# abdenlab/giql

Hardware: AMD Instinct MI355X
Metric: overlap-pairs/sec, 10Mx100M INTERSECTS inner join (higher is better)
Workload: dtype int32

## Files before the change

### giql_amd/csrc/giql_hip.hip

```cpp
#include <hip/hip_runtime.h>
#include <chrono>
#include <atomic>
#include <sys/mman.h>
#include <utility>
#if defined(__SSE2__)
#include <emmintrin.h>
#endif
#include <mutex>
#include <thread>
#include <stdarg.h>
#include <stdio.h>
#include <stdlib.h>
#include <string.h>

#include <vector>

#include "../../include/giql_hip.h"
#include "aux_kernels.hip.h"
#include "take_kernels.hip.h"
#include "select_kernels.hip.h"
#include "cluster_kernels.hip.h"
#include "disjoin_kernels.hip.h"
#include "contain_kernels.hip.h"
#include "dev_common.hip.h"
#include "join_kernels.hip.h"
#include "onesweep.hip.h"
#include "bucket_sort.hip.h"
#include "radix_sort.hip.h"
#include "scan.hip.h"
#include "probe_kernels.hip.h"

using namespace giql;

static thread_local char g_err[512] = "";

static int set_err(int code, const char* fmt, ...) {
  va_list ap;
  va_start(ap, fmt);
  vsnprintf(g_err, sizeof(g_err), fmt, ap);
  va_end(ap);
  return code;
}

#define HIP_TRY(expr)                                                                     \
  do {                                                                                    \
    hipError_t _e = (expr);                                                               \
    if (_e != hipSuccess)                                                                 \
      return set_err(GIQL_ERR_HIP, "%s failed: %s (%s:%d)", #expr, hipGetErrorString(_e), \
                     __FILE__, __LINE__);                                                 \
  } while (0)

#define GIQL_TRY(expr)      \
  do {                      \
    int _rc = (expr);       \
    if (_rc != GIQL_OK) return _rc; \
  } while (0)

#ifndef GIQL_RC_ITEMS
#define GIQL_RC_ITEMS 1
#endif
constexpr int RC_ITEMS_C2 = GIQL_RC_ITEMS;
#ifndef GIQL_FILL_ITEMS
#define GIQL_FILL_ITEMS 16
#endif
constexpr int FILL_ITEMS_C2 = GIQL_FILL_ITEMS;

#ifndef GIQL_STREAM_GRID
#define GIQL_STREAM_GRID 16384u
#endif

static inline size_t align_up(size_t x, size_t a) { return (x + a - 1) / a * a; }
static inline u32 cdiv(u64 a, u64 b) { return (u32)((a + b - 1) / b); }

struct SortBufs {
  u32* key[2];
  u32* end[2];
  u32* rid[2];
};

struct InnerState {
  SortBufs sa, sb;
  u32 nt1 = 0, nt2 = 0;
  int c1_items = C1_ITEMS_MAX;
  u32* wlo1 = nullptr;
  u64* c1_base = nullptr;
  bool c1_fill = false;
  u32 *lo1 = nullptr, *cnt1 = nullptr;
  u64* off1 = nullptr;
  u32* wlo2 = nullptr;
  u32* lo2 = nullptr;
  u32* cnt2 = nullptr;
  u64* off2 = nullptr;
  int uniform = 0;
};

constexpr size_t C1_SMALL_ROWS = (size_t)4 << 20;
constexpr u64 OVERLAP_MAX_ROWS = (u64)4 << 20;

struct Switches {
  bool classic_sort = false;
  int os_variant = 0;
  int os_order = 2;
  u32 os_help_after = OS_HELP_AFTER;
  int inject_timeout = 0;
  bool no_uniform = false;
  bool no_span_hist = false;
  bool no_coarse_b = false;
  double coarse_max_group_rows = 8.0;
  bool no_fuse_count = false;
  bool no_local_sort = false;
  u64 local_min_rows = 1u << 21;
  double local_min_bucket_rows = 300.0;
  double local_max_bucket_rows = 2800.0;
  bool no_narrow = false;
  int force_bits = 0;
};

struct Guesses {
  bool local_sort = true;
  int os_order = 2;
  int inject_timeout = 0;
  u64 last_span = 0;
  bool last_no_irr = false;
  bool nearest_two_sorts = false;
  int nearest_aligned = -1;
  bool spec_valid = false;
  int spec_form = 0;
  i64 spec_len = 0;
  bool spec_aligned = false;
  bool spec_fuse_len_ok = false;
  bool spec_sorted[2] = {false, false};
  bool row_spec_valid = false;
  i64 row_spec_len = 0;
  int spec_misses = 0;
  int local_resorts = 0;
  int order_fallbacks = 0;
};

struct CallState {
  bool prezeroed = false;
  bool first_unstable = false;
  u32* span_hist_dirty[2] = {nullptr, nullptr};
  int force_local = 0;
  int index_bits = 16;
  bool used_sorted[2] = {false, false};
  bool last_sort_local = false;
  int last_local_bits = 16;
  bool count_fused = false;
  bool bucket_join = false;
};

struct InnerPlan {
  bool planned = false;
  bool plan_is_join = false;
  bool swapped = false;
  int32_t* fuse_a = nullptr;
  int32_t* fuse_b = nullptr;
  u64 fuse_cap = 0;
  bool fuse_done = false;
  giql_side side_a, side_b;
  u32 n_a = 0, n_b = 0;
  int n_chrom = 0;
  u64 n_reg = 0, n_irr = 0, n_c1 = 0;
  InnerState inner;
  u32* irr_a_list = nullptr;
  u32* irr_b_list = nullptr;
  u64* irr_off = nullptr;
};

struct DisjoinPlan {
  bool planned = false;
  giql_side target;
  u64 total = 0;
  i64* chrom_base = nullptr;
  u64* off = nullptr;
  u32* lo_first = nullptr;
  u32* bp = nullptr;
  u64* n_bp = nullptr;
  u32* ncov = nullptr;
  u32* cbp = nullptr;
};

struct ContainPlan {
  bool planned = false;
  giql_side outer, inner;
  u32 n_o = 0, n_i = 0;
  int form = 0;
  u64 n_cand = 0;
  u64 n_reg = 0, n_irr = 0;
  u32 n_tiles = 0;
  SortBufs so, si;
  u32* lo = nullptr;
  u64* coff = nullptr;
  u32* ct_part = nullptr;
  u64* tile_off = nullptr;
  u32* irr_o_list = nullptr;
  u32* irr_i_list = nullptr;
  u64* irr_off = nullptr;
};

struct giql_hip_ctx {
  explicit giql_hip_ctx(const Switches& s) : sw(s) {
    guess.local_sort = !s.no_local_sort;
    guess.os_order = s.os_order;
    guess.inject_timeout = s.inject_timeout;
  }
  const Switches sw;
  Guesses guess;
  CallState call;
  InnerPlan plan;
  DisjoinPlan dj;
  ContainPlan ct;

  int device = 0;
  int n_cu = 256;
  char* arena = nullptr;
  size_t arena_cap = 0;
  DevMeta* d_meta = nullptr;
  DevMeta* h_meta = nullptr;
  u32* part = nullptr;
  size_t part_cap = 0;
  void* stage_out = nullptr;
  size_t stage_out_cap = 0;
  char* xplan = nullptr;
  size_t xplan_cap = 0;
  char* ct_buf = nullptr;
  size_t ct_buf_cap = 0;
  u64* d_scratch64 = nullptr;
  hipStream_t side_stream = nullptr;
  hipEvent_t ev_fork = nullptr, ev_join = nullptr;
  u32* bucket_qwin = nullptr;
  u32* bucket_bnd = nullptr;
  u32* bucket_big = nullptr;

  int profiling = 0;
  int profile_phase = GIQL_PH_SORT_SCATTER;
  std::vector<hipEvent_t> ev_pool;
  struct Span {
    int phase;
    hipEvent_t a, b;
  };
  std::vector<Span> spans;
  size_t ev_used = 0;
  giql_hip_stats stats;
};

struct Carver {
  char* base;
  size_t off = 0;
  template <typename T>
  T* take(size_t n) {
    off = align_up(off, 256);
    T* p = base ? reinterpret_cast<T*>(base + off) : nullptr;
    off += n * sizeof(T);
    return p;
  }
};

static int grow_buffer(void** buf, size_t* cap, size_t need, size_t want, hipStream_t stream, const char* what) {
  if (need <= *cap) return GIQL_OK;
  HIP_TRY(hipStreamSynchronize(stream));
  if (*buf) HIP_TRY(hipFree(*buf));
  *buf = nullptr;
  *cap = 0;
  const hipError_t e = hipMalloc(buf, want);
  if (e != hipSuccess)
    return set_err(GIQL_ERR_NOMEM, "hipMalloc(%zu bytes) for %s failed: %s", want, what, hipGetErrorString(e));
  *cap = want;
  return GIQL_OK;
}

static int ensure_arena(giql_hip_ctx* ctx, size_t bytes, hipStream_t stream) {
  if (bytes <= ctx->arena_cap) return GIQL_OK;
  ctx->plan.planned = false;
  ctx->dj.planned = false;
  ctx->ct.planned = false;
  const size_t want = align_up(bytes + bytes / 8, (size_t)1 << 20);
  GIQL_TRY(grow_buffer((void**)&ctx->arena, &ctx->arena_cap, bytes, want, stream, "the workspace"));
  if (getenv("GIQL_HIP_DEBUG_ADDR")) fprintf(stderr, "[giql_hip] arena %p + %zu bytes\n", (void*)ctx->arena, want);
  return GIQL_OK;
}

static int grow_part(giql_hip_ctx* ctx, size_t words, hipStream_t stream) {
  return grow_buffer((void**)&ctx->part, &ctx->part_cap, words * sizeof(u32), (words + words / 4) * sizeof(u32), stream,
                     "the fill partition");
}

template <typename Carve>
static int claim_arena(giql_hip_ctx* ctx, hipStream_t stream, Carve&& carve) {
  ctx->plan.planned = false;
  ctx->dj.planned = false;
  ctx->ct.planned = false;
  GIQL_TRY(ensure_arena(ctx, carve(nullptr), stream));
  carve(ctx->arena);
  return GIQL_OK;
}

struct Phase {
  giql_hip_ctx* ctx;
  hipStream_t stream;
  int phase;
  hipEvent_t a = nullptr, b = nullptr;
  Phase(giql_hip_ctx* c, hipStream_t s, int ph, int launches = 1) : ctx(c), stream(s), phase(ph) {
    ctx->stats.phase_launches[ph] += launches;
    if (!ctx->profiling || (ctx->profiling == 2 && ph != ctx->profile_phase)) return;
    while (ctx->ev_used + 2 > ctx->ev_pool.size()) {
      hipEvent_t e;
      if (hipEventCreate(&e) != hipSuccess) return;
      ctx->ev_pool.push_back(e);
    }
    a = ctx->ev_pool[ctx->ev_used++];
    b = ctx->ev_pool[ctx->ev_used++];
    (void)hipEventRecord(a, stream);
  }
  ~Phase() {
    if (!a) return;
    (void)hipEventRecord(b, stream);
    ctx->spans.push_back({phase, a, b});
  }
};

static void reset_stats(giql_hip_ctx* ctx) {
  memset(&ctx->stats, 0, sizeof(ctx->stats));
  ctx->call = CallState{};
  ctx->spans.clear();
  ctx->ev_used = 0;
}

static int begin_call(giql_hip_ctx* ctx) {
  HIP_TRY(hipSetDevice(ctx->device));
  ctx->ct.planned = false;
  reset_stats(ctx);
  return GIQL_OK;
}

static int check_side(const giql_side* s, const char* name);
static int begin_pair_call(giql_hip_ctx* ctx, const giql_side* a, const giql_side* b, int32_t n_chrom) {
  GIQL_TRY(check_side(a, "a"));
  GIQL_TRY(check_side(b, "b"));
  if (n_chrom < 0) return set_err(GIQL_ERR_INVALID, "n_chrom < 0");
  GIQL_TRY(begin_call(ctx));
  ctx->stats.n_a = a->n;
  ctx->stats.n_b = b->n;
  return GIQL_OK;
}

struct PrezeroGuard {
  giql_hip_ctx* c;
  ~PrezeroGuard() {
    c->call.prezeroed = false;
    c->call.first_unstable = false;
  }
};

struct ForceLocal {
  giql_hip_ctx* c;
  ForceLocal(giql_hip_ctx* ctx, int v) : c(ctx) { c->call.force_local = v; }
  ~ForceLocal() {
    c->call.force_local = 0;
    c->call.index_bits = 16;
  }
};

static void collect_spans(giql_hip_ctx* ctx) {
  if (!ctx->profiling) return;
  for (auto& s : ctx->spans) {
    float ms = 0.f;
    if (hipEventElapsedTime(&ms, s.a, s.b) == hipSuccess) ctx->stats.phase_ms[s.phase] += ms;
  }
  ctx->spans.clear();
  ctx->ev_used = 0;
  float t = 0.f;
  for (int i = 0; i < GIQL_PH_N; i++) t += ctx->stats.phase_ms[i];
  ctx->stats.total_ms = t;
  ctx->stats.profiled = 1;
}

static int check_side(const giql_side* s, const char* name) {
  if (!s) return set_err(GIQL_ERR_INVALID, "side %s is NULL", name);
  if (s->n < 0 || s->n > 0x7FFFFFF0ll)
    return set_err(GIQL_ERR_INVALID, "side %s: n=%lld outside [0, 2^31-16]", name, (long long)s->n);
  if (s->n > 0 && (!s->chrom || !s->start || !s->end))
    return set_err(GIQL_ERR_INVALID, "side %s: NULL column buffer", name);
  if (s->start_off < -1 || s->start_off > 0 || s->end_off < -1 || s->end_off > 1)
    return set_err(GIQL_ERR_INVALID, "side %s: canonical offsets (%d,%d) outside {0,-1}x{+1,0,-1}",
                   name, s->start_off, s->end_off);
  return GIQL_OK;
}

static SideView view_of(const giql_side& s) {
  SideView v;
  v.chrom = s.chrom;
  v.start = s.start;
  v.end = s.end;
  v.n = (u32)s.n;
  v.start_off = s.start_off;
  v.end_off = s.end_off;
  return v;
}

static int post_launch(const char* what) {
  hipError_t e = hipGetLastError();
  if (e != hipSuccess)
    return set_err(GIQL_ERR_HIP, "kernel launch failed in %s: %s", what, hipGetErrorString(e));
  return GIQL_OK;
}

template <typename TOut>
static int run_scan(giql_hip_ctx* ctx, hipStream_t st, int phase, const u32* in, u64 n, TOut* out,
                    u64* bsums, u64* total_out, u64* total_out2 = nullptr) {
  if (n == 0) {
    if (total_out) HIP_TRY(hipMemsetAsync(total_out, 0, sizeof(u64), st));
    if (total_out2) HIP_TRY(hipMemsetAsync(total_out2, 0, sizeof(u64), st));
    return GIQL_OK;
  }
  const u32 nb = cdiv(n, SCAN_TILE);
  Phase ph(ctx, st, phase, 3);
  hipLaunchKernelGGL(k_scan_reduce, dim3(nb), dim3(SCAN_NT), 0, st, in, n, bsums);
  hipLaunchKernelGGL(k_scan_spine, dim3(1), dim3(1024), 0, st, bsums, nb, total_out, total_out2);
  hipLaunchKernelGGL((k_scan_down<TOut>), dim3(nb), dim3(SCAN_NT), 0, st, in, n, bsums, out);
  return post_launch("scan");
}

static int run_scan_diff(giql_hip_ctx* ctx, hipStream_t st, int phase, u32* hi, u32* lo, u64 n, const u32* n_irr,
                         u64* out, u64* bsums, u64* total_out, u64* total_out2) {
  const u32 nb = cdiv(n, SCAN_TILE);
  Phase ph(ctx, st, phase, 3);
  hipLaunchKernelGGL(k_scan_reduce_diff, dim3(nb), dim3(SCAN_NT), 0, st, hi, lo, n, n_irr, bsums);
  hipLaunchKernelGGL(k_scan_spine, dim3(1), dim3(1024), 0, st, bsums, nb, total_out, total_out2);
  hipLaunchKernelGGL(k_scan_down_diff, dim3(nb), dim3(SCAN_NT), 0, st, hi, lo, n, n_irr, bsums, out);
  return post_launch("scan (bounds)");
}

static int run_scan_chain(giql_hip_ctx* ctx, hipStream_t st, int phase, const u32* hi, const u32* lo, u64 n,
                          const u32* n_irr, u64* out, u64* chain_status, u64* total_out2, u32* part, u32 tile_log2,
                          u32 part_cap) {
  const u32 nb = cdiv(n, SC_TILE);
  Phase ph(ctx, st, phase, 1);
  hipLaunchKernelGGL(k_scan_chain_diff, dim3(nb), dim3(SC_NT), 0, st, hi, lo, (u32)n, n_irr, chain_status,
                     reinterpret_cast<u32*>(chain_status + nb + 1), out, total_out2, part, tile_log2, part_cap);
  return post_launch("scan (chained)");
}

struct LinBufs {
  int* gmin;
  int* gmax;
  i64* chrom_base;
  u32* chrom_first;
  int* len_part;
  u32* abase = nullptr;
  u32* top_partial = nullptr;
  u32* top_partial2 = nullptr;
  u32* hist_partial2 = nullptr;
};

static inline int sort_local_bits(const giql_hip_ctx* ctx, size_t n);
static inline bool sort_is_local(const giql_hip_ctx* ctx, size_t n) { return sort_local_bits(ctx, n) != 0; }

static int run_spans(giql_hip_ctx* ctx, hipStream_t st, const giql_side& a, const giql_side& b,
                     int n_chrom, const LinBufs& lb, int hist_side = -1, u32* hist_partial = nullptr) {
  const bool hist = hist_side >= 0 && hist_partial && lb.abase && lb.top_partial &&
                    n_chrom <= MM_HIST_CHROMS && (hist_side ? b.n : a.n) > 0;
  const bool hist2 = hist && lb.hist_partial2 && lb.top_partial2 && ctx->call.prezeroed && (hist_side ? a.n : b.n) > 0;
  if (hist && !ctx->call.prezeroed) {
    HIP_TRY(hipMemsetAsync(hist_partial, 0, (size_t)LIN_HIST_REPLICAS * 1024 * sizeof(u32), st));
    HIP_TRY(hipMemsetAsync(lb.top_partial, 0, (size_t)LIN_HIST_REPLICAS * MM_TOP_WORDS * sizeof(u32), st));
  }
  Phase ph(ctx, st, GIQL_PH_SPAN, 4);
  hipLaunchKernelGGL(k_init_minmax, dim3(cdiv((u64)n_chrom + 1, 256)), dim3(256), 0, st, lb.gmin,
                     lb.gmax, n_chrom, ctx->d_meta);
  const size_t lds = n_chrom <= MM_LDS_CHROMS ? (size_t)n_chrom * 2 * sizeof(int) : 0;
  const giql_side* sides[2] = {&a, &b};
  int nblk[2] = {0, 0};
  if (a.n > 0 && b.n > 0) {
    MmSide ms[2];
    const double tot = (double)a.n + (double)b.n;
    for (int k = 0; k < 2; k++) {
      const giql_side& s = *sides[k];
      const bool with_hist = hist && (k == hist_side || hist2);
      u32* const hp = k == hist_side ? hist_partial : lb.hist_partial2;
      if (with_hist) ctx->call.span_hist_dirty[k] = hp;
      u32 grid = (u32)((double)MM_MAX_BLOCKS * (double)s.n / tot + 0.5);
      const u32 need = cdiv((u64)s.n, (u64)MM_NT_HIST * 4);
      if (grid > need) grid = need;
      if (grid < 1) grid = 1;
      nblk[k] = (int)grid;
      ms[k].chrom = s.chrom;
      ms[k].start = s.start;
      ms[k].end = s.end;
      ms[k].n = (i64)s.n;
      ms[k].len_bias = s.end_off - s.start_off;
      ms[k].start_off = with_hist ? s.start_off : 0;
      ms[k].hist = !with_hist ? 0 : (sort_local_bits(ctx, (size_t)s.n) == 16 ? 2 : 1);
      ms[k].nblk = grid;
      ms[k].hist_partial = with_hist ? hp : nullptr;
      ms[k].top_partial = with_hist ? (k == hist_side ? lb.top_partial : lb.top_partial2) : nullptr;
    }
    hipLaunchKernelGGL((k_chrom_minmax2<MM_NT_HIST>), dim3(ms[0].nblk + ms[1].nblk), dim3(MM_NT_HIST), lds, st, ms[0], ms[1],
                       n_chrom, lb.gmin, lb.gmax, ctx->d_meta, lb.len_part);
  } else
  for (int k = 0; k < 2; k++) {
    const giql_side& s = *sides[k];
    if (s.n == 0) continue;
    const bool with_hist = hist && (k == hist_side || hist2);
    u32* const hp = k == hist_side ? hist_partial : lb.hist_partial2;
    if (with_hist) ctx->call.span_hist_dirty[k] = hp;
    u32* const tp = k == hist_side ? lb.top_partial : lb.top_partial2;
    u32 grid = cdiv((u64)s.n, (u64)(with_hist ? MM_NT_HIST : MM_NT) * MM_ITEMS);
    if (grid > (u32)MM_MAX_BLOCKS) grid = MM_MAX_BLOCKS;
    nblk[k] = (int)grid;
    if (with_hist && sort_local_bits(ctx, (size_t)s.n) == 16)
      hipLaunchKernelGGL((k_chrom_minmax<2, MM_NT_HIST>), dim3(grid), dim3(MM_NT_HIST), lds, st, s.chrom, s.start, s.end,
                         (i64)s.n, n_chrom, lb.gmin, lb.gmax, ctx->d_meta, s.end_off - s.start_off, k,
                         lb.len_part, s.start_off, hp, tp);
    else if (with_hist)
      hipLaunchKernelGGL((k_chrom_minmax<1, MM_NT_HIST>), dim3(grid), dim3(MM_NT_HIST), lds, st, s.chrom, s.start, s.end,
                         (i64)s.n, n_chrom, lb.gmin, lb.gmax, ctx->d_meta, s.end_off - s.start_off, k,
                         lb.len_part, s.start_off, hp, tp);
    else
      hipLaunchKernelGGL((k_chrom_minmax<0, MM_NT>), dim3(grid), dim3(MM_NT), lds, st, s.chrom, s.start, s.end,
                         (i64)s.n, n_chrom, lb.gmin, lb.gmax, ctx->d_meta, s.end_off - s.start_off, k,
                         lb.len_part, 0, (u32*)nullptr, (u32*)nullptr);
  }
  int omin = a.start_off, omax = a.start_off;
  const int offs[3] = {a.end_off, b.start_off, b.end_off};
  for (int k = 0; k < 3; k++) {
    if (offs[k] < omin) omin = offs[k];
    if (offs[k] > omax) omax = offs[k];
  }
  hipLaunchKernelGGL(k_chrom_offsets, dim3(1), dim3(256), 0, st, lb.gmin, lb.gmax, n_chrom, omin,
                     omax, lb.chrom_base, lb.chrom_first, ctx->d_meta, lb.len_part, nblk[0], nblk[1],
                     hist ? 1 : 0, lb.abase);
  return post_launch("spans");
}

static int run_linearize(giql_hip_ctx* ctx, hipStream_t st, const giql_side& s, int n_chrom,
                         const LinBufs& lb, u32* keys, u32* ends, u32* irr_list, int which,
                         int keep_irregular, u32* hist_partial = nullptr, u32* gbase = nullptr,
                         u32* hist_end = nullptr, u32* gbase_end = nullptr, bool skip_end = false) {
  if (s.n == 0) return GIQL_OK;
  const int* end_col = skip_end ? (const int*)nullptr : s.end;
  bool dirty = false;
  for (int k = 0; k < 2; k++)
    if (hist_partial && ctx->call.span_hist_dirty[k] == hist_partial) {
      dirty = true;
      ctx->call.span_hist_dirty[k] = nullptr;
    }
  if (hist_partial && (!ctx->call.prezeroed || dirty))
    HIP_TRY(hipMemsetAsync(hist_partial, 0, (size_t)LIN_HIST_REPLICAS * 1024 * sizeof(u32), st));
  if (hist_end && !ctx->call.prezeroed)
    HIP_TRY(hipMemsetAsync(hist_end, 0, (size_t)LIN_HIST_REPLICAS * 1024 * sizeof(u32), st));
  Phase ph(ctx, st, GIQL_PH_LINEARIZE, hist_partial ? 2 : 1);
  u32 grid = cdiv((u64)s.n, LIN_NT);
  if (grid > (u32)LIN_MAX_BLOCKS) grid = LIN_MAX_BLOCKS;
  if (hist_end)
    hipLaunchKernelGGL((k_linearize<true>), dim3(grid), dim3(LIN_NT), 0, st, s.chrom, s.start, end_col,
                       (u32)s.n, s.start_off, s.end_off, n_chrom, lb.chrom_base, keys, ends, irr_list,
                       ctx->d_meta, which, keep_irregular, hist_partial, hist_end);
  else
    hipLaunchKernelGGL((k_linearize<false>), dim3(grid), dim3(LIN_NT), 0, st, s.chrom, s.start, end_col,
                       (u32)s.n, s.start_off, s.end_off, n_chrom, lb.chrom_base, keys, ends, irr_list,
                       ctx->d_meta, which, keep_irregular, hist_partial, (u32*)nullptr);
  if (hist_partial)
    hipLaunchKernelGGL(k_digit_offsets, dim3(4), dim3(256), 0, st, hist_partial,
                       (u32)LIN_HIST_REPLICAS, gbase);
  if (hist_end)
    hipLaunchKernelGGL(k_digit_offsets, dim3(4), dim3(256), 0, st, hist_end, (u32)LIN_HIST_REPLICAS,
                       gbase_end);
  return post_launch("linearize");
}

static inline size_t os_pass_words(size_t n) {
  return (size_t)cdiv(n ? n : 1, OS_MIN_TILE) * OS_BINS + 16;
}
static inline size_t os_pass_stride(const giql_hip_ctx* ctx, size_t n) {
  return ctx->sw.os_variant == 0 ? (size_t)cdiv(n ? n : 1, 8192) * OS_BINS + 16 : os_pass_words(n);
}

template <int NT, int ITEMS>
static void launch_onesweep(giql_hip_ctx* ctx, hipStream_t st, SortBufs& sb, int src, int dst, bool first,
                            u32 n, int shift, const u32* gbase, u32* status, DevMeta* meta, int unstable = 0) {
  const u32 grid = cdiv(n, NT * ITEMS);
  u32* claim = status + os_pass_stride(ctx, n) - 16;
  const u32* rin = (first || !sb.rid[0]) ? (const u32*)nullptr : sb.rid[src];
  const int mode = (sb.rid[0] ? 1 : 0) | (sb.end[0] ? 2 : 0);
#define GIQL_OS_LAUNCH(M)                                                                            \
  hipLaunchKernelGGL((k_onesweep<M, NT, ITEMS>), dim3(grid), dim3(NT), 0, st, sb.key[src],           \
                     sb.end[0] ? sb.end[src] : (const u32*)nullptr, rin, sb.key[dst],                 \
                     sb.end[0] ? sb.end[dst] : (u32*)nullptr, sb.rid[0] ? sb.rid[dst] : (u32*)nullptr, \
                     n, shift, gbase, status, claim, meta, ctx->guess.os_order, ctx->sw.os_help_after, (const u32*)nullptr, 0u, 0u,  \
                     unstable)
  switch (mode) {
    case 0: GIQL_OS_LAUNCH(0); break;
    case 1: GIQL_OS_LAUNCH(1); break;
    case 2: GIQL_OS_LAUNCH(2); break;
    default: GIQL_OS_LAUNCH(3); break;
  }
#undef GIQL_OS_LAUNCH
}

static inline int density_bits(const giql_hip_ctx* ctx, double per_bucket) {
  int w = 16;
  while (per_bucket > ctx->sw.local_max_bucket_rows && w > BS_MIN_WBITS && !ctx->sw.no_narrow) {
    per_bucket *= 0.5;
    w--;
  }
  return per_bucket <= ctx->sw.local_max_bucket_rows ? w : 0;
}

static inline int sort_local_bits(const giql_hip_ctx* ctx, size_t n) {
  if (ctx->call.force_local > 0 && ctx->bucket_bnd && ctx->sw.os_variant == 0) return ctx->call.index_bits;
  if (ctx->call.force_local < 0) return 0;
  if (!(ctx->guess.local_sort && ctx->bucket_bnd && ctx->sw.os_variant == 0 && n >= ctx->sw.local_min_rows)) return 0;
  const double span = ctx->guess.last_span ? (double)ctx->guess.last_span : 3.2e9;
  double per_bucket = (double)n * 65536.0 / span;
  if (per_bucket < ctx->sw.local_min_bucket_rows) return 0;
  if (ctx->sw.force_bits) return ctx->sw.force_bits;
  return density_bits(ctx, per_bucket);
}
static inline int local_passes(int wbits) { return wbits == 16 ? 2 : 3; }

struct FuseCount {
  BsFuse dev;
  u32 nq_total;
  const u32* irr_q;
  const u32* gbq3;
  u32 key_mask;
  const int* len_max_q;
  u32* zero_ptr;
  u32 zero_words;
  bool join = false;
  bool general = false;
  const int* len_max_u = nullptr;
};

static int64_t bucket_stage_fused_bytes(u32 n, const FuseCount& fuse);
static void launch_bucket_stage_fused(giql_hip_ctx* ctx, hipStream_t st, SortBufs& sb, u32 n, const u32* gbase,
                                      const FuseCount& fuse_in, int wbits = 16) {
  FuseCount fuse = fuse_in;
  fuse.dev.wbits = (u32)wbits;
  const u32 BS_BUCKETS = bs_n_buckets((u32)wbits);
  ctx->stats.phase_bytes[GIQL_PH_SORT_LOCAL] += bucket_stage_fused_bytes(n, fuse);
  ctx->call.count_fused = true;
  ctx->call.bucket_join = fuse.join;
  ctx->call.last_local_bits = wbits;
  {
    Phase ph(ctx, st, GIQL_PH_COUNT, 1);
    hipLaunchKernelGGL(k_bucket_bounds_fused, dim3(cdiv((u64)3 * BS_BUCKETS + 1, 256)), dim3(256), 0, st, sb.key[0], n,
                       gbase + 3 * OS_BINS, ctx->bucket_bnd, ctx->bucket_big, fuse.dev, fuse.nq_total, fuse.irr_q,
                       fuse.gbq3, fuse.key_mask, fuse.len_max_q, fuse.zero_ptr, fuse.zero_words, fuse.len_max_u);
  }
  const bool w16 = wbits == 16;
#define GIQL_BSF_LAUNCH(P, F, W)                                                                                    \
  hipLaunchKernelGGL((k_bucket_sort<P, F, W>), dim3(BS_BUCKETS), dim3(BS_NT), 0, st, sb.key[0],                      \
                     (P) == 3 ? sb.end[0] : (u32*)nullptr, sb.rid[0], ctx->bucket_bnd, ctx->d_meta, ctx->bucket_big, \
                     fuse.dev)
  if (fuse.general) {
    {
      Phase ph(ctx, st, GIQL_PH_SORT_LOCAL, 1);
      if (w16) GIQL_BSF_LAUNCH(3, 3, true); else GIQL_BSF_LAUNCH(3, 3, false);
    }
    Phase ph(ctx, st, GIQL_PH_AUX, 1);
    hipLaunchKernelGGL((k_bucket_sort_big<3, 3>), dim3(ctx->n_cu), dim3(BS_NT), 0, st, sb.key[0], sb.end[0], sb.rid[0],
                       sb.key[1], sb.end[1], sb.rid[1], ctx->bucket_bnd, ctx->bucket_big, fuse.dev);
    return;
  }
  {
    Phase ph(ctx, st, GIQL_PH_SORT_LOCAL, 1);
    if (fuse.join) {
      if (w16) GIQL_BSF_LAUNCH(1, 2, true); else GIQL_BSF_LAUNCH(1, 2, false);
    } else {
      if (w16) GIQL_BSF_LAUNCH(1, 1, true); else GIQL_BSF_LAUNCH(1, 1, false);
    }
  }
#undef GIQL_BSF_LAUNCH
  {
    Phase ph(ctx, st, GIQL_PH_AUX, 1);
    if (fuse.join)
      hipLaunchKernelGGL((k_bucket_sort_big<1, 2>), dim3(ctx->n_cu), dim3(BS_NT), 0, st, sb.key[0], (u32*)nullptr,
                         sb.rid[0], sb.key[1], (u32*)nullptr, sb.rid[1], ctx->bucket_bnd, ctx->bucket_big, fuse.dev);
    else
      hipLaunchKernelGGL((k_bucket_sort_big<1, 1>), dim3(ctx->n_cu), dim3(BS_NT), 0, st, sb.key[0], (u32*)nullptr,
                         sb.rid[0], sb.key[1], (u32*)nullptr, sb.rid[1], ctx->bucket_bnd, ctx->bucket_big, fuse.dev);
  }
}
static int64_t bucket_stage_fused_bytes(u32 n, const FuseCount& fuse) {
  if (fuse.general) return (int64_t)12 * n + (int64_t)12 * fuse.nq_total;
  return fuse.join ? (int64_t)8 * n + (int64_t)12 * fuse.nq_total : (int64_t)12 * n + (int64_t)16 * fuse.nq_total;
}

static int run_sort_onesweep(giql_hip_ctx* ctx, hipStream_t st, SortBufs& sb, u32 n,
                             const u32* gbase, u32* status, bool keep_rids = false,
                             const giql_side* keygen = nullptr, const u32* abase = nullptr,
                             int skip_digits = 0, const FuseCount* fuse = nullptr, bool presorted = false) {
  if (n == 0) return GIQL_OK;
  if (presorted) {
    const int mode = (sb.rid[0] ? 1 : 0) | (sb.end[0] ? 2 : 0);
    const int wbits_pre = sort_local_bits(ctx, n);
    const bool local_fused = fuse && mode == (fuse->general ? 3 : 1) && wbits_pre != 0;
    {
      Phase ph(ctx, st, GIQL_PH_SORT_SCATTER, 1);
      u32 grid = cdiv(n, 256 * 8);
      if (grid > GIQL_STREAM_GRID) grid = GIQL_STREAM_GRID;
      if (keygen) {
        ctx->stats.phase_bytes[GIQL_PH_SORT_SCATTER] += (int64_t)4 * n * ((mode & 2 ? 3 : 2) + 1 + (mode & 1) + (mode & 2 ? 1 : 0));
        const u32 so = (u32)keygen->start_off, eo = (u32)keygen->end_off;
        switch (mode) {
          case 0: hipLaunchKernelGGL(k_keygen_stream<0>, dim3(grid), dim3(256), 0, st, keygen->chrom, keygen->start, keygen->end, n, abase, so, eo, sb.key[0], (u32*)nullptr, (u32*)nullptr); break;
          case 1: hipLaunchKernelGGL(k_keygen_stream<1>, dim3(grid), dim3(256), 0, st, keygen->chrom, keygen->start, keygen->end, n, abase, so, eo, sb.key[0], (u32*)nullptr, sb.rid[0]); break;
          case 2: hipLaunchKernelGGL(k_keygen_stream<2>, dim3(grid), dim3(256), 0, st, keygen->chrom, keygen->start, keygen->end, n, abase, so, eo, sb.key[0], sb.end[0], (u32*)nullptr); break;
          default: hipLaunchKernelGGL(k_keygen_stream<3>, dim3(grid), dim3(256), 0, st, keygen->chrom, keygen->start, keygen->end, n, abase, so, eo, sb.key[0], sb.end[0], sb.rid[0]); break;
        }
      } else if (sb.rid[0] && !keep_rids) {
        ctx->stats.phase_bytes[GIQL_PH_SORT_SCATTER] += (int64_t)4 * n;
        hipLaunchKernelGGL(k_iota, dim3(grid), dim3(256), 0, st, sb.rid[0], n);
      }
      GIQL_TRY(post_launch("sorted input (no sort)"));
    }
    if (!local_fused) return GIQL_OK;
    ctx->call.last_sort_local = true;
    launch_bucket_stage_fused(ctx, st, sb, n, gbase, *fuse, wbits_pre);
    return post_launch("bucket stage (sorted input, fused count)");
  }
  const int wbits = sort_local_bits(ctx, n);
  const bool local = wbits != 0;
  if (local) ctx->call.last_sort_local = true;
  if (local) skip_digits = 0;
  const int n_pass = local ? local_passes(wbits) : 4 - skip_digits;
  const int first_digit = local ? 4 - n_pass : skip_digits;
  const size_t per_pass = os_pass_stride(ctx, n);
  if (!ctx->call.prezeroed) HIP_TRY(hipMemsetAsync(status, 0, n_pass * per_pass * sizeof(u32), st));
  {
    Phase ph(ctx, st, GIQL_PH_SORT_SCATTER, n_pass);
    for (int pass = 0; pass < n_pass; pass++) {
      const int src = pass & 1, dst = src ^ 1;
      const int digit = first_digit + pass;
      u32* stat = status + pass * per_pass;
      const bool first = pass == 0 && !keep_rids;
      const u32* gb = gbase + digit * OS_BINS;
      {
        const int w_out = 1 + (sb.rid[0] ? 1 : 0) + (sb.end[0] ? 1 : 0);
        const int w_in = (pass == 0 && keygen) ? 2 + (sb.end[0] ? 1 : 0)
                                               : 1 + ((sb.rid[0] && !first) ? 1 : 0) + (sb.end[0] ? 1 : 0);
        ctx->stats.phase_bytes[GIQL_PH_SORT_SCATTER] += (int64_t)4 * (w_in + w_out) * n;
      }
      const int unstable = (pass == 0 && !keep_rids && ctx->call.first_unstable) ? 1 : 0;
      if (pass == 0 && keygen) {
        const u32 grid = cdiv(n, 1024 * 8);
        u32* claim = stat + per_pass - 16;
        if (sb.end[0])
          hipLaunchKernelGGL((k_onesweep<3, 1024, 8, true>), dim3(grid), dim3(1024), 0, st,
                             reinterpret_cast<const u32*>(keygen->start), reinterpret_cast<const u32*>(keygen->end),
                             reinterpret_cast<const u32*>(keygen->chrom), sb.key[dst], sb.end[dst], sb.rid[dst], n,
                             digit * 8, gb, stat, claim, ctx->d_meta, ctx->guess.os_order, ctx->sw.os_help_after, abase,
                             (u32)keygen->start_off, (u32)keygen->end_off, unstable);
        else
          hipLaunchKernelGGL((k_onesweep<1, 1024, 8, true>), dim3(grid), dim3(1024), 0, st,
                             reinterpret_cast<const u32*>(keygen->start), reinterpret_cast<const u32*>(keygen->chrom),
                             (const u32*)nullptr, sb.key[dst], (u32*)nullptr, sb.rid[dst], n, digit * 8, gb, stat, claim,
                             ctx->d_meta, ctx->guess.os_order, ctx->sw.os_help_after, abase, (u32)keygen->start_off, 0u, unstable);
        continue;
      }
      switch (ctx->sw.os_variant) {
        case 1: launch_onesweep<512, 8>(ctx, st, sb, src, dst, first, n, digit * 8, gb, stat, ctx->d_meta, unstable); break;
        case 2: launch_onesweep<512, 16>(ctx, st, sb, src, dst, first, n, digit * 8, gb, stat, ctx->d_meta, unstable); break;
        case 3: launch_onesweep<256, 16>(ctx, st, sb, src, dst, first, n, digit * 8, gb, stat, ctx->d_meta, unstable); break;
        case 4: launch_onesweep<1024, 4>(ctx, st, sb, src, dst, first, n, digit * 8, gb, stat, ctx->d_meta, unstable); break;
        case 5: case 7: launch_onesweep<1024, 12>(ctx, st, sb, src, dst, first, n, digit * 8, gb, stat, ctx->d_meta, unstable); break;
        default: launch_onesweep<1024, 8>(ctx, st, sb, src, dst, first, n, digit * 8, gb, stat, ctx->d_meta, unstable); break;
      }
    }
  }
  if (n_pass & 1) {
    u32* t;
    t = sb.key[0], sb.key[0] = sb.key[1], sb.key[1] = t;
    t = sb.end[0], sb.end[0] = sb.end[1], sb.end[1] = t;
    t = sb.rid[0], sb.rid[0] = sb.rid[1], sb.rid[1] = t;
  }
  if (local) {
    const int mode = (sb.rid[0] ? 1 : 0) | (sb.end[0] ? 2 : 0);
    if (fuse && mode == (fuse->general ? 3 : 1)) {
      launch_bucket_stage_fused(ctx, st, sb, n, gbase, *fuse, wbits);
      return post_launch("onesweep sort (fused count)");
    }
    BsFuse bw;
    bw.wbits = (u32)wbits;
    ctx->call.last_local_bits = wbits;
    const u32 BS_BUCKETS = bs_n_buckets((u32)wbits);
    HIP_TRY(hipMemsetAsync(ctx->bucket_big, 0, sizeof(u32), st));
    Phase ph(ctx, st, GIQL_PH_SORT_LOCAL, 3);
    ctx->stats.phase_bytes[GIQL_PH_SORT_LOCAL] +=
        (int64_t)8 * (1 + (sb.rid[0] ? 1 : 0) + (sb.end[0] ? 1 : 0)) * n;
    hipLaunchKernelGGL(k_bucket_bounds, dim3(cdiv((u64)BS_BUCKETS + 1, 256)), dim3(256), 0, st, sb.key[0], n,
                       gbase + 3 * OS_BINS, ctx->bucket_bnd, (u32)wbits);
#define GIQL_BS_LAUNCH(M)                                                                              \
  if (wbits == 16)                                                                                     \
    hipLaunchKernelGGL((k_bucket_sort<M, 0, true>), dim3(BS_BUCKETS), dim3(BS_NT), 0, st, sb.key[0],   \
                       sb.end[0] ? sb.end[0] : (u32*)nullptr, sb.rid[0] ? sb.rid[0] : (u32*)nullptr,    \
                       ctx->bucket_bnd, ctx->d_meta, ctx->bucket_big, bw);                             \
  else                                                                                                 \
  hipLaunchKernelGGL((k_bucket_sort<M>), dim3(BS_BUCKETS), dim3(BS_NT), 0, st, sb.key[0],              \
                     sb.end[0] ? sb.end[0] : (u32*)nullptr, sb.rid[0] ? sb.rid[0] : (u32*)nullptr,      \
                     ctx->bucket_bnd, ctx->d_meta, ctx->bucket_big, bw);                               \
  hipLaunchKernelGGL((k_bucket_sort_big<M>), dim3(ctx->n_cu), dim3(BS_NT), 0, st, sb.key[0],           \
                     sb.end[0] ? sb.end[0] : (u32*)nullptr, sb.rid[0] ? sb.rid[0] : (u32*)nullptr,      \
                     sb.key[1], sb.end[0] ? sb.end[1] : (u32*)nullptr, sb.rid[0] ? sb.rid[1] : (u32*)nullptr, \
                     ctx->bucket_bnd, ctx->bucket_big, bw)
    switch (mode) {
      case 0: GIQL_BS_LAUNCH(0); break;
      case 1: GIQL_BS_LAUNCH(1); break;
      case 2: GIQL_BS_LAUNCH(2); break;
      default: GIQL_BS_LAUNCH(3); break;
    }
#undef GIQL_BS_LAUNCH
  }
  return post_launch("onesweep sort");
}

static inline void adopt_by_end(SortBufs& owner, const SortBufs& by_end) {
  for (int k = 0; k < 2; k++) {
    owner.end[k] = by_end.key[k];
    owner.key[k] = by_end.end[k];
    owner.rid[k] = by_end.rid[k];
  }
}

static int run_sort(giql_hip_ctx* ctx, hipStream_t st, SortBufs& sb, u32 n, u32* tile_hist,
                    u64* bsums) {
  if (n == 0) return GIQL_OK;
  const u32 n_tiles = cdiv(n, RS_TILE);
  for (int pass = 0; pass < 4; pass++) {
    const int src = pass & 1, dst = src ^ 1;
    const int shift = pass * 8;
    {
      Phase ph(ctx, st, GIQL_PH_SORT_HIST);
      hipLaunchKernelGGL(k_radix_hist, dim3(n_tiles), dim3(RS_NT), 0, st, sb.key[src], n, shift,
                         n_tiles, tile_hist);
    }
    GIQL_TRY(run_scan<u32>(ctx, st, GIQL_PH_SORT_SCAN, tile_hist, (u64)n_tiles * RS_BINS, tile_hist,
                           bsums, nullptr));
    {
      Phase ph(ctx, st, GIQL_PH_SORT_SCATTER);
      if (sb.end[0]) {
        hipLaunchKernelGGL((k_radix_scatter<true>), dim3(n_tiles), dim3(RS_NT), 0, st, sb.key[src],
                           sb.end[src], pass == 0 ? (const u32*)nullptr : sb.rid[src], sb.key[dst],
                           sb.end[dst], sb.rid[dst], n, shift, n_tiles, tile_hist);
      } else {
        hipLaunchKernelGGL((k_radix_scatter<false>), dim3(n_tiles), dim3(RS_NT), 0, st, sb.key[src],
                           (const u32*)nullptr, (const u32*)nullptr, sb.key[dst], (u32*)nullptr,
                           (u32*)nullptr, n, shift, n_tiles, tile_hist);
      }
    }
  }
  return post_launch("radix sort");
}

static int run_pmax(giql_hip_ctx* ctx, hipStream_t st, const u32* in, u32 n, u32* out, u32* bmax) {
  if (n == 0) return GIQL_OK;
  const u32 nb = cdiv(n, PM_TILE);
  Phase ph(ctx, st, GIQL_PH_AUX, 3);
  hipLaunchKernelGGL(k_pmax_reduce, dim3(nb), dim3(PM_NT), 0, st, in, n, bmax);
  hipLaunchKernelGGL(k_pmax_spine, dim3(1), dim3(1024), 0, st, bmax, nb);
  hipLaunchKernelGGL(k_pmax_down, dim3(nb), dim3(PM_NT), 0, st, in, n, bmax, out);
  return post_launch("prefix max");
}

static int read_meta(giql_hip_ctx* ctx, hipStream_t st) {
  HIP_TRY(hipMemcpyAsync(ctx->h_meta, ctx->d_meta, sizeof(DevMeta), hipMemcpyDeviceToHost, st));
  HIP_TRY(hipStreamSynchronize(st));
  int status = ctx->h_meta->status;
  if (ctx->guess.inject_timeout > 0 && ctx->guess.os_order != 0 && status == 0 && --ctx->guess.inject_timeout == 0)
    status = ctx->h_meta->status = GIQL_ERR_HIP;
  if (status == GIQL_STATUS_RESORT)
    return set_err(GIQL_STATUS_RESORT, "a 16-bit key bucket holds more than %u rows", BS_CAP);
  if (status == GIQL_ERR_HIP)
    return set_err(GIQL_ERR_HIP, "onesweep look-back timed out (tile order %d)", ctx->guess.os_order);
  if (status == GIQL_ERR_CHROM)
    return set_err(GIQL_ERR_CHROM, "a chrom id is outside [0, n_chrom)");
  if (status == GIQL_ERR_SPAN)
    return set_err(GIQL_ERR_SPAN,
                   "linearised coordinate span %llu does not fit 32 bits; shard the chromosomes "
                   "into groups (giql_amd.shard) and join each group",
                   (unsigned long long)ctx->h_meta->total_span);
  if (status != 0) return set_err(status, "device reported status %d", status);
  return GIQL_OK;
}

static void common_sizes(Carver& c, int n_chrom, LinBufs& lb) {
  lb.gmin = c.take<int>((size_t)n_chrom);
  lb.gmax = c.take<int>((size_t)n_chrom);
  lb.chrom_base = c.take<i64>((size_t)n_chrom);
  lb.chrom_first = c.take<u32>((size_t)n_chrom + 1);
  lb.len_part = c.take<int>((size_t)2 * MM_MAX_BLOCKS * 2);
}

static void sort_sizes(Carver& c, size_t n, SortBufs& sb, bool payload) {
  for (int k = 0; k < 2; k++) {
    sb.key[k] = c.take<u32>(n);
    sb.end[k] = payload ? c.take<u32>(n) : nullptr;
    sb.rid[k] = payload ? c.take<u32>(n) : nullptr;
  }
}

static inline int row_skip(const giql_hip_ctx* ctx, size_t nb) {
  if (ctx->guess.last_span == 0) return 1;
  return (double)nb * 65536.0 / (double)ctx->guess.last_span <= 1024.0 ? 2 : 1;
}

static inline bool coarse_b_ok(const giql_hip_ctx* ctx, size_t nb) {
  if (ctx->sw.no_coarse_b || ctx->guess.last_span == 0 || sort_is_local(ctx, nb)) return false;
  return (double)nb * 256.0 / (double)ctx->guess.last_span <= ctx->sw.coarse_max_group_rows;
}

struct SideChain {
  giql_hip_ctx* ctx;
  hipStream_t main;
  bool active = false, joined = false;
  SideChain(giql_hip_ctx* c, hipStream_t m, size_t n_small) : ctx(c), main(m) {
    if (!c->side_stream || n_small == 0 || n_small > OVERLAP_MAX_ROWS) return;
    if (sort_is_local(c, n_small)) return;
    if (hipEventRecord(c->ev_fork, m) != hipSuccess) return;
    if (hipStreamWaitEvent(c->side_stream, c->ev_fork, 0) != hipSuccess) return;
    active = true;
  }
  hipStream_t stream() const { return active ? ctx->side_stream : main; }
  int join() {
    if (active && !joined) {
      joined = true;
      HIP_TRY(hipEventRecord(ctx->ev_join, ctx->side_stream));
      HIP_TRY(hipStreamWaitEvent(main, ctx->ev_join, 0));
    }
    return GIQL_OK;
  }
  ~SideChain() {
    if (active && !joined) (void)hipStreamSynchronize(ctx->side_stream);
  }
};

constexpr int GIQL_STATUS_GUESS_MISSED = -101;
constexpr int MAX_GUESS_MISSES = 2;

template <typename F>
static int with_order_fallback(giql_hip_ctx* ctx, F&& call) {
  int misses = 0;
  for (;;) {
    const int rc = call();
    if (rc == GIQL_STATUS_GUESS_MISSED) {
      if (++misses > MAX_GUESS_MISSES)
        return set_err(GIQL_ERR_STATE, "internal: more than %d guesses missed in one call", MAX_GUESS_MISSES);
      continue;
    }
    if (rc == GIQL_STATUS_RESORT && ctx && ctx->guess.local_sort) {
      ctx->guess.local_sort = false;
      ctx->guess.local_resorts++;
      misses = 0;
      continue;
    }
    if (rc == GIQL_ERR_HIP && ctx && ctx->guess.os_order != 0 && ctx->h_meta && ctx->h_meta->status == GIQL_ERR_HIP) {
      ctx->guess.os_order = 0;
      ctx->guess.order_fallbacks++;
      misses = 0;
      continue;
    }
    return rc;
  }
}

static inline i64 uniform_len_b(const DevMeta& m) {
  return (m.len_min_b == m.len_max_b && m.len_max_b > 0) ? (i64)m.len_max_b : 0;
}

static int row_form_guess(giql_hip_ctx* ctx, hipStream_t st, i64& uni_len, bool& speculated) {
  uni_len = 0;
  speculated = false;
  if (ctx->sw.no_uniform) return GIQL_OK;
  if (ctx->guess.row_spec_valid) {
    uni_len = ctx->guess.row_spec_len;
    speculated = true;
    return GIQL_OK;
  }
  GIQL_TRY(read_meta(ctx, st));
  uni_len = uniform_len_b(*ctx->h_meta);
  ctx->guess.last_span = ctx->h_meta->total_span;
  return GIQL_OK;
}

static bool row_form_settled(giql_hip_ctx* ctx, i64 uni_len, bool speculated) {
  if (ctx->sw.no_uniform) return true;
  const i64 actual = uniform_len_b(*ctx->h_meta);
  const bool ok = !(speculated && uni_len != 0 && actual != uni_len);
  ctx->guess.row_spec_valid = ok;
  ctx->guess.row_spec_len = actual;
  return ok;
}

static void parse_flag(const char* v, void* f) { *(bool*)f = atoi(v) != 0; }
static void parse_int(const char* v, void* f) { *(int*)f = atoi(v); }
static void parse_u32(const char* v, void* f) { *(u32*)f = (u32)strtoul(v, nullptr, 10); }
static void parse_classic(const char* v, void* f) { *(bool*)f = strcmp(v, "classic") == 0; }
static void parse_positive(const char* v, void* f) {
  if (atof(v) > 0) *(double*)f = atof(v);
}
static void parse_nonnegative(const char* v, void* f) {
  if (atof(v) >= 0) *(double*)f = atof(v);
}
static void parse_local_bits(const char* v, void* f) {
  if (atoi(v) >= BS_MIN_WBITS && atoi(v) <= 16) *(int*)f = atoi(v);
}
static void parse_local_min_rows(const char* v, void* f) {
  Switches& s = *(Switches*)f;
  s.local_min_rows = strtoull(v, nullptr, 10);
  s.local_max_bucket_rows = 1e30;
  s.local_min_bucket_rows = 0.0;
}

static Switches read_switches() {
  Switches s;
  const struct {
    const char* name;
    void (*parse)(const char*, void*);
    void* field;
  } table[] = {
      {"GIQL_HIP_SORT", parse_classic, &s.classic_sort},
      {"GIQL_HIP_OS_VARIANT", parse_int, &s.os_variant},
      {"GIQL_HIP_OS_ORDER", parse_int, &s.os_order},
      {"GIQL_HIP_OS_HELP_AFTER", parse_u32, &s.os_help_after},
      {"GIQL_HIP_INJECT_TIMEOUT", parse_int, &s.inject_timeout},
      {"GIQL_HIP_NO_UNIFORM", parse_flag, &s.no_uniform},
      {"GIQL_HIP_NO_SPAN_HIST", parse_flag, &s.no_span_hist},
      {"GIQL_HIP_NO_COARSE_B", parse_flag, &s.no_coarse_b},
      {"GIQL_HIP_COARSE_MAX_GROUP_ROWS", parse_positive, &s.coarse_max_group_rows},
      {"GIQL_HIP_NO_FUSE_COUNT", parse_flag, &s.no_fuse_count},
      {"GIQL_HIP_NO_LOCAL_SORT", parse_flag, &s.no_local_sort},
      {"GIQL_HIP_LOCAL_MIN_ROWS", parse_local_min_rows, &s},
      {"GIQL_HIP_LOCAL_MIN_BUCKET_ROWS", parse_nonnegative, &s.local_min_bucket_rows},
      {"GIQL_HIP_LOCAL_MAX_BUCKET_ROWS", parse_positive, &s.local_max_bucket_rows},
      {"GIQL_HIP_NO_NARROW_BUCKETS", parse_flag, &s.no_narrow},
      {"GIQL_HIP_LOCAL_BITS", parse_local_bits, &s.force_bits},
  };
  for (const auto& row : table)
    if (const char* v = getenv(row.name)) row.parse(v, row.field);
  return s;
}

extern "C" {

int giql_hip_abi_version(void) { return GIQL_HIP_ABI_VERSION; }

const char* giql_hip_last_error(void) { return g_err; }

int giql_hip_device_count(int* n_devices) {
  if (!n_devices) return set_err(GIQL_ERR_INVALID, "n_devices is NULL");
  int n = 0;
  HIP_TRY(hipGetDeviceCount(&n));
  *n_devices = n;
  return GIQL_OK;
}

int giql_hip_create(int device, giql_hip_ctx** out) {
  if (!out) return set_err(GIQL_ERR_INVALID, "out is NULL");
  *out = nullptr;
  int n = 0;
  HIP_TRY(hipGetDeviceCount(&n));
  if (device < 0 || device >= n)
    return set_err(GIQL_ERR_INVALID, "device %d not in [0,%d)", device, n);
  HIP_TRY(hipSetDevice(device));
  giql_hip_ctx* ctx = new (std::nothrow) giql_hip_ctx(read_switches());
  if (!ctx) return set_err(GIQL_ERR_NOMEM, "out of host memory");
  ctx->device = device;
  memset(&ctx->stats, 0, sizeof(ctx->stats));
  {
    hipDeviceProp_t prop;
    if (hipGetDeviceProperties(&prop, device) == hipSuccess && prop.multiProcessorCount > 0)
      ctx->n_cu = prop.multiProcessorCount;
  }
  hipError_t e = hipMalloc((void**)&ctx->d_meta, sizeof(DevMeta));
  if (e == hipSuccess) e = hipHostMalloc((void**)&ctx->h_meta, sizeof(DevMeta), hipHostMallocDefault);
  if (e == hipSuccess) e = hipMalloc((void**)&ctx->d_scratch64, 64);
  if (e == hipSuccess &&
      (hipStreamCreateWithFlags(&ctx->side_stream, hipStreamNonBlocking) != hipSuccess ||
       hipEventCreateWithFlags(&ctx->ev_fork, hipEventDisableTiming) != hipSuccess ||
       hipEventCreateWithFlags(&ctx->ev_join, hipEventDisableTiming) != hipSuccess))
    ctx->side_stream = nullptr;
  if (e == hipSuccess) e = hipMalloc((void**)&ctx->bucket_bnd, ((size_t)BS_MAX_BUCKETS + 16) * sizeof(u32));
  if (e == hipSuccess) e = hipMalloc((void**)&ctx->bucket_big, ((size_t)BS_MAX_BUCKETS + 16) * sizeof(u32));
  if (e == hipSuccess) e = hipMalloc((void**)&ctx->bucket_qwin, ((size_t)2 * BS_MAX_BUCKETS + 16) * sizeof(u32));
  if (e != hipSuccess) {
    giql_hip_destroy(ctx);
    return set_err(GIQL_ERR_HIP, "context allocation failed: %s", hipGetErrorString(e));
  }
  *out = ctx;
  return GIQL_OK;
}

int giql_hip_destroy(giql_hip_ctx* ctx) {
  if (!ctx) return GIQL_OK;
  (void)hipSetDevice(ctx->device);
  (void)hipDeviceSynchronize();
  for (auto e : ctx->ev_pool) (void)hipEventDestroy(e);
  if (ctx->arena) (void)hipFree(ctx->arena);
  if (ctx->part) (void)hipFree(ctx->part);
  if (ctx->stage_out) (void)hipFree(ctx->stage_out);
  if (ctx->d_meta) (void)hipFree(ctx->d_meta);
  if (ctx->d_scratch64) (void)hipFree(ctx->d_scratch64);
  if (ctx->ev_fork) (void)hipEventDestroy(ctx->ev_fork);
  if (ctx->ev_join) (void)hipEventDestroy(ctx->ev_join);
  if (ctx->side_stream) (void)hipStreamDestroy(ctx->side_stream);
  if (ctx->bucket_bnd) (void)hipFree(ctx->bucket_bnd);
  if (ctx->bucket_big) (void)hipFree(ctx->bucket_big);
  if (ctx->bucket_qwin) (void)hipFree(ctx->bucket_qwin);
  if (ctx->xplan) (void)hipFree(ctx->xplan);
  if (ctx->ct_buf) (void)hipFree(ctx->ct_buf);
  if (ctx->h_meta) (void)hipHostFree(ctx->h_meta);
  delete ctx;
  return GIQL_OK;
}

int giql_hip_reserve(giql_hip_ctx* ctx, int64_t bytes) {
  if (!ctx || bytes < 0) return set_err(GIQL_ERR_INVALID, "bad ctx/bytes");
  HIP_TRY(hipSetDevice(ctx->device));
  return ensure_arena(ctx, (size_t)bytes, nullptr);
}

int giql_hip_set_profiling(giql_hip_ctx* ctx, int enabled) {
  if (!ctx) return set_err(GIQL_ERR_INVALID, "ctx is NULL");
  if (enabled >= 16 && enabled < 16 + GIQL_PH_N) {
    ctx->profiling = 2;
    ctx->profile_phase = enabled - 16;
    return GIQL_OK;
  }
  ctx->profiling = enabled < 0 ? 0 : (enabled > 2 ? 1 : enabled);
  ctx->profile_phase = GIQL_PH_SORT_SCATTER;
  return GIQL_OK;
}

int giql_hip_get_stats(giql_hip_ctx* ctx, giql_hip_stats* out) {
  if (!ctx || !out) return set_err(GIQL_ERR_INVALID, "ctx/out is NULL");
  if (ctx->profiling && !ctx->spans.empty()) {
    HIP_TRY(hipSetDevice(ctx->device));
    HIP_TRY(hipEventSynchronize(ctx->spans.back().b));
    collect_spans(ctx);
  }
  ctx->stats.workspace_bytes = (int64_t)ctx->arena_cap;
  *out = ctx->stats;
  out->reserved = (ctx->stats.reserved & 0x1F) | (ctx->call.last_sort_local ? 0x20 : 0) |
                  (ctx->guess.local_resorts ? 0x40 : 0) | (ctx->plan.swapped ? 0x80 : 0) | ((ctx->guess.os_order & 0x7F) << 8) |
                  (ctx->call.count_fused ? 0x8000 : 0) | ((ctx->call.used_sorted[0] || ctx->call.used_sorted[1]) ? (int32_t)0x80000000u : 0) |
                  ((ctx->guess.order_fallbacks & 0x7FF) << 16) | (((16 - ctx->call.last_local_bits) & 3) << 27) |
                  (ctx->call.bucket_join ? (1 << 29) : 0) |
                  (ctx->plan.fuse_done ? (1 << 30) : 0);
  return GIQL_OK;
}

struct PlanSide {
  const giql_side* side = nullptr;
  size_t n = 0;
  int label = 0;
  SortBufs* sort = nullptr;
  u32 *hist = nullptr, *gbase = nullptr;
  u32* status = nullptr;
  u32* irr_list = nullptr;
  const u32* irr = nullptr;
  const int* len_max = nullptr;
  int32_t* out_row = nullptr;
};

struct InnerScratch {
  LinBufs lb;
  u32 *tile_hist = nullptr, *irr_cnt = nullptr, *top_partial_q = nullptr;
  u32 *hist[2] = {nullptr, nullptr}, *gbase[2] = {nullptr, nullptr};
  u32 *os_status = nullptr, *os_status2 = nullptr;
  u64 *bsums = nullptr, *bsums1 = nullptr, *scan_chain = nullptr;
  size_t zero_off = 0, zero_end = 0;
  int big_passes_zeroed = 0;
};

struct InnerAttempt {
  bool onesweep = false;
  int big_side = 0;
  bool speculated = false;
  int form = 0;
  i64 uni_len = 0;
  bool want_hist = false;
  bool want_hist_q = false;
  bool aligned = false;
  bool keygen_u = false;
  bool keygen_q = false;
  bool keygen_g = false;
  bool presorted[2] = {false, false};
  bool no_irr = false;
  bool fuse_len_ok = false;
  int q_skip = 0;
  bool fuse_cnt = false;
  bool early_fill = false;
  bool join_in_buckets = false;
  bool general_join = false;

  bool count_fused() const { return fuse_cnt || general_join; }
  bool bucket_join() const { return join_in_buckets || general_join; }
};

static inline int len_min_of(const DevMeta& m, int label) { return label ? m.len_min_b : m.len_min_a; }
static inline int len_max_of(const DevMeta& m, int label) { return label ? m.len_max_b : m.len_max_a; }
static inline u32 skip_mask(int q_skip) { return q_skip == 2 ? 0xFFFF0000u : (q_skip == 1 ? 0xFFFFFF00u : 0xFFFFFFFFu); }

static void decide_form(const DevMeta& m, size_t na, size_t nb, bool no_uniform, int& form, i64& len) {
  const bool ub = m.len_min_b == m.len_max_b && m.len_max_b > 0;
  const bool ua = m.len_min_a == m.len_max_a && m.len_max_a > 0;
  form = 0;
  len = 0;
  if (no_uniform) return;
  if (ub && (!ua || nb >= na)) {
    form = 1;
    len = m.len_max_b;
  } else if (ua) {
    form = 2;
    len = m.len_max_a;
  }
}

static bool fuse_len_ok(const DevMeta& m, int form) {
  if (form != 0) return len_max_of(m, form == 1 ? 0 : 1) <= (int)BS_FUSE_WCAP;
  return m.len_max_a <= (int)BS_FUSE_WCAP && m.len_max_b <= (int)BS_FUSE_WCAP;
}

static size_t carve_inner(giql_hip_ctx* ctx, char* base, size_t na, size_t nb, int n_chrom, bool onesweep,
                          InnerScratch& W) {
  InnerState& S = ctx->plan.inner;
  const size_t nq = na + nb, n_max = na > nb ? na : nb;
  const size_t n_tiles_max = cdiv(n_max, RS_TILE);
  const size_t scan_max = (nq > n_tiles_max * RS_BINS ? nq : n_tiles_max * RS_BINS);
  constexpr u32 TQ2 = RC_NT * RC_ITEMS_C2;
  Carver c{base};
  common_sizes(c, n_chrom, W.lb);
  sort_sizes(c, na, S.sa, true);
  sort_sizes(c, nb, S.sb, true);
  if (onesweep) {
    c.off = align_up(c.off, 256);
    W.zero_off = c.off;
    W.hist[0] = c.take<u32>((size_t)LIN_HIST_REPLICAS * 1024);
    W.hist[1] = c.take<u32>((size_t)LIN_HIST_REPLICAS * 1024);
    W.lb.top_partial = c.take<u32>((size_t)LIN_HIST_REPLICAS * MM_TOP_WORDS);
    W.top_partial_q = c.take<u32>((size_t)LIN_HIST_REPLICAS * MM_TOP_WORDS);
    W.gbase[0] = c.take<u32>(1024);
    W.gbase[1] = c.take<u32>(1024);
    W.lb.abase = c.take<u32>(MM_HIST_CHROMS);
    W.os_status2 = c.take<u32>(4 * os_pass_words(na < nb ? na : nb));
    c.off = align_up(c.off, 256);
    W.zero_end = c.off;
    W.os_status = c.take<u32>(4 * os_pass_words(n_max));
  } else {
    W.tile_hist = c.take<u32>(n_tiles_max * RS_BINS);
  }
  W.bsums = c.take<u64>(cdiv(scan_max, SCAN_TILE) + 2);
  S.wlo1 = c.take<u32>((size_t)S.nt1 + 2 + (S.c1_fill ? cdiv(nb, TQ2) : 0));
  S.c1_base = c.take<u64>((size_t)S.nt1 + 2);
  const size_t n1 = S.c1_fill ? nb : 0;
  S.lo1 = c.take<u32>(n1);
  S.cnt1 = c.take<u32>(n1);
  S.off1 = c.take<u64>(n1 + 1);
  W.bsums1 = c.take<u64>(cdiv(n1 ? n1 : 1, SCAN_TILE) + 2);
  const size_t nq2 = ctx->sw.no_uniform ? na : n_max;
  S.wlo2 = c.take<u32>((size_t)cdiv(nq2, TQ2) + 2);
  S.cnt2 = c.take<u32>(nq2);
  S.lo2 = c.take<u32>(nq2);
  S.off2 = c.take<u64>(nq2 + 1);
  W.scan_chain = c.take<u64>((size_t)cdiv(nq2, SCAN_TILE) + 4);
  ctx->plan.irr_a_list = c.take<u32>(na);
  ctx->plan.irr_b_list = c.take<u32>(nb);
  W.irr_cnt = c.take<u32>(nq);
  ctx->plan.irr_off = c.take<u64>(nq + 1);
  return c.off;
}

static int zero_inner_scratch(giql_hip_ctx* ctx, hipStream_t st, InnerScratch& W, size_t n_max) {
  const int passes = sort_is_local(ctx, n_max) ? local_passes(sort_local_bits(ctx, n_max)) : 4;
  const size_t stride = os_pass_stride(ctx, n_max);
  if (W.big_passes_zeroed == 0) {
    HIP_TRY(hipMemsetAsync(ctx->arena + W.zero_off, 0,
                           (W.zero_end - W.zero_off) + (size_t)passes * stride * sizeof(u32), st));
    ctx->call.prezeroed = true;
  } else if (W.big_passes_zeroed < passes) {
    HIP_TRY(hipMemsetAsync(W.os_status + (size_t)W.big_passes_zeroed * stride, 0,
                           (size_t)(passes - W.big_passes_zeroed) * stride * sizeof(u32), st));
  } else {
    return GIQL_OK;
  }
  W.big_passes_zeroed = passes;
  return GIQL_OK;
}

static void bind_status(const InnerScratch& W, PlanSide& x, PlanSide& y) {
  const bool x_small = x.n <= y.n;
  x.status = x_small ? W.os_status2 : W.os_status;
  y.status = x_small ? W.os_status : W.os_status2;
}

static int begin_attempt(giql_hip_ctx* ctx, hipStream_t st, PlanSide& A, PlanSide& B, int n_chrom, InnerScratch& W,
                         InnerAttempt& T) {
  const Guesses& g = ctx->guess;
  PlanSide& big = T.big_side ? B : A;
  PlanSide& other = T.big_side ? A : B;
  const int big_form = T.big_side ? 1 : 2;
  T.speculated = T.onesweep && g.spec_valid;
  T.no_irr = T.speculated && g.last_no_irr;
  T.want_hist = T.onesweep && !ctx->sw.no_span_hist && ctx->sw.os_variant == 0 && n_chrom <= MM_HIST_CHROMS;
  if (T.want_hist && T.speculated)
    T.want_hist = g.spec_aligned && (g.spec_form == big_form || (g.spec_form == 0 && g.last_no_irr));
  T.want_hist_q = T.want_hist && T.no_irr && g.spec_form == big_form && other.n > 0;
  if (T.want_hist_q) {
    W.lb.hist_partial2 = other.hist;
    W.lb.top_partial2 = W.top_partial_q;
  }
  GIQL_TRY(run_spans(ctx, st, *A.side, *B.side, n_chrom, W.lb, T.want_hist ? T.big_side : -1, big.hist));
  if (T.speculated) {
    T.form = g.spec_form;
    T.uni_len = g.spec_len;
    T.aligned = T.want_hist;
    T.fuse_len_ok = g.spec_fuse_len_ok;
    T.presorted[0] = g.spec_sorted[0];
    T.presorted[1] = g.spec_sorted[1];
  } else if (T.onesweep) {
    GIQL_TRY(read_meta(ctx, st));
    const DevMeta& m = *ctx->h_meta;
    decide_form(m, A.n, B.n, ctx->sw.no_uniform, T.form, T.uni_len);
    T.aligned = T.want_hist && m.aligned_ok != 0;
    T.fuse_len_ok = fuse_len_ok(m, T.form);
    T.presorted[0] = m.unsorted_a == 0;
    T.presorted[1] = m.unsorted_b == 0;
    const int expected_bits = sort_local_bits(ctx, big.n);
    ctx->guess.last_span = m.total_span;
    if (expected_bits == 16 && sort_local_bits(ctx, big.n) != 16) T.aligned = false;
    GIQL_TRY(zero_inner_scratch(ctx, st, W, big.n));
  }
  T.keygen_u = T.aligned && T.form == big_form;
  T.keygen_q = T.keygen_u && T.want_hist_q;
  T.keygen_g = T.aligned && T.form == 0 && (T.speculated ? g.last_no_irr : len_min_of(*ctx->h_meta, T.big_side) > 0);
  return GIQL_OK;
}

static int span_digit_offsets(giql_hip_ctx* ctx, hipStream_t st, const LinBufs& lb, u32* hist, u32* gbase,
                              u32* hist2, u32* gbase2, const char* what) {
  Phase ph(ctx, st, GIQL_PH_LINEARIZE, 2);
  if (hist2) {
    hipLaunchKernelGGL(k_fold_top2, dim3(MM_HIST_CHROMS, 2), dim3(256), 0, st, lb.top_partial, lb.top_partial2,
                       lb.abase, hist, hist2);
    hipLaunchKernelGGL(k_digit_offsets2, dim3(4, 2), dim3(256), 0, st, hist, hist2, (u32)LIN_HIST_REPLICAS, gbase,
                       gbase2);
  } else {
    hipLaunchKernelGGL(k_fold_top, dim3(MM_HIST_CHROMS), dim3(256), 0, st, lb.top_partial, lb.abase, hist);
    hipLaunchKernelGGL(k_digit_offsets, dim3(4), dim3(256), 0, st, hist, (u32)LIN_HIST_REPLICAS, gbase);
  }
  return post_launch(what);
}

struct FuseQuery {
  const SortBufs* sort;
  size_t n;
  const u32* irr;
  const u32* gbase;
  const int* len_max;
};
struct FuseTarget {
  int32_t *row_q, *row_s;
  u64 cap;
};
static inline FuseQuery fuse_query(const PlanSide& q) { return FuseQuery{q.sort, q.n, q.irr, q.gbase, q.len_max}; }

static FuseCount make_fuse_count(giql_hip_ctx* ctx, const FuseQuery& q, i64 lo_off, u32 key_mask,
                                 const FuseTarget* join, bool general, const int* len_max_u, u32* zero_ptr) {
  FuseCount fc = {};
  fc.join = join != nullptr;
  fc.general = general;
  fc.zero_ptr = zero_ptr;
  fc.dev.qkey = q.sort->key[0];
  fc.dev.qend = q.sort->end[0];
  fc.dev.qwin = ctx->bucket_qwin;
  fc.dev.lo_off = lo_off;
  if (join) {
    fc.dev.qrid = q.sort->rid[0];
    fc.dev.row_q = join->row_q;
    fc.dev.row_s = join->row_s;
    fc.dev.cap = join->cap;
    fc.dev.cursor = reinterpret_cast<unsigned long long*>(&ctx->d_meta->n_out);
  }
  fc.nq_total = (u32)q.n;
  fc.irr_q = q.irr;
  fc.gbq3 = q.gbase + 3 * OS_BINS;
  fc.key_mask = key_mask;
  fc.len_max_q = q.len_max;
  fc.len_max_u = general ? len_max_u : nullptr;
  return fc;
}

static int finish_bucket_join(giql_hip_ctx* ctx, hipStream_t st) {
  GIQL_TRY(read_meta(ctx, st));
  ctx->plan.n_c1 = 0;
  ctx->plan.n_reg = ctx->h_meta->n_out;
  ctx->plan.fuse_done = ctx->h_meta->irr_a + ctx->h_meta->irr_b == 0 && ctx->plan.n_reg <= ctx->plan.fuse_cap;
  ctx->stats.phase_bytes[GIQL_PH_SORT_LOCAL] += (int64_t)8 * (int64_t)ctx->plan.n_reg;
  return GIQL_OK;
}

static int plan_uniform(giql_hip_ctx* ctx, hipStream_t st, int n_chrom, PlanSide& Q, PlanSide& U, InnerScratch& W,
                        InnerAttempt& T) {
  InnerState& S = ctx->plan.inner;
  const LinBufs& lb = W.lb;
  SortBufs& sq = *Q.sort;
  SortBufs& su = *U.sort;
  su.end[0] = su.end[1] = nullptr;
  bind_status(W, Q, U);
  T.fuse_cnt = !ctx->sw.no_fuse_count && sort_is_local(ctx, U.n) && T.fuse_len_ok;
  const int q_len_max = len_max_of(*ctx->h_meta, Q.label);
  if (T.keygen_u) {
    GIQL_TRY(span_digit_offsets(ctx, st, lb, U.hist, U.gbase, T.keygen_q ? Q.hist : nullptr, Q.gbase,
                                "digit offsets (span histogram)"));
  }
  SideChain sc(ctx, st, (Q.n <= U.n && !T.fuse_cnt) ? Q.n : 0);
  if (!T.keygen_q) {
    GIQL_TRY(run_linearize(ctx, sc.stream(), *Q.side, n_chrom, lb, sq.key[0], sq.end[0], Q.irr_list, Q.label, 0,
                           Q.hist, Q.gbase));
  }
  if (!T.keygen_u) {
    GIQL_TRY(run_linearize(ctx, st, *U.side, n_chrom, lb, su.key[0], nullptr, U.irr_list, U.label, 0, U.hist,
                           U.gbase, nullptr, nullptr, true));
  }
  T.q_skip = (T.no_irr && !sort_is_local(ctx, Q.n)) ? 1 : 0;
  const int wb_u = sort_local_bits(ctx, U.n);
  if (T.q_skip && T.fuse_cnt && wb_u == 16) T.q_skip = 2;
  const u32 q_mask = skip_mask(T.q_skip);
  GIQL_TRY(run_sort_onesweep(ctx, sc.stream(), sq, (u32)Q.n, Q.gbase, Q.status, false,
                             T.keygen_q ? Q.side : nullptr, lb.abase, T.q_skip, nullptr, T.presorted[Q.label]));
  constexpr u32 T2 = FILL_NT * FILL_ITEMS_C2;
  static_assert((T2 & (T2 - 1)) == 0, "fill tiles are a power of two (k_scan_chain_diff shifts)");
  const u64 nt_cap64 = (ctx->plan.fuse_cap + T2 - 1) / T2;
  const bool offered = Q.out_row && T.no_irr && ctx->plan.fuse_cap > 0;
  T.early_fill = offered && nt_cap64 <= 0x7FFFFFF0ull && ((size_t)nt_cap64 + 2) * sizeof(u32) <= ctx->part_cap;
  const double win_keys = T.q_skip == 2 ? 3.0 * 65536.0 + (double)T.uni_len
                                        : (double)(1u << (wb_u ? wb_u : 16)) + 512.0 + (double)T.uni_len +
                                              (double)(q_len_max > 0 ? q_len_max : 0);
  T.join_in_buckets = T.fuse_cnt && offered && ctx->guess.last_span > 0 &&
                      (double)Q.n * win_keys / (double)ctx->guess.last_span <= 0.75 * (double)BJ_WCAP;
  FuseCount fc = {};
  if (T.fuse_cnt) {
    const FuseTarget out{Q.out_row, U.out_row, ctx->plan.fuse_cap};
    fc = make_fuse_count(ctx, fuse_query(Q), 1 - T.uni_len, q_mask, T.join_in_buckets ? &out : nullptr, false, nullptr,
                         reinterpret_cast<u32*>(W.scan_chain));
    fc.zero_words = (u32)(2 * (cdiv(Q.n, SC_TILE) + 2));
    fc.dev.lo_out = S.lo2;
    fc.dev.hi_out = S.cnt2;
  }
  GIQL_TRY(run_sort_onesweep(ctx, st, su, (u32)U.n, U.gbase, U.status, false, T.keygen_u ? U.side : nullptr, lb.abase,
                             0, T.fuse_cnt ? &fc : nullptr, T.presorted[U.label]));
  GIQL_TRY(sc.join());
  constexpr u32 TQ = RC_NT * RC_ITEMS_C2;
  S.nt2 = cdiv(Q.n, TQ);
  if (T.join_in_buckets) return finish_bucket_join(ctx, st);
  bool part_done = false;
  if (T.fuse_cnt) {
    u32 log2_t2 = 0;
    while ((1u << log2_t2) < T2) log2_t2++;
    GIQL_TRY(run_scan_chain(ctx, st, GIQL_PH_SCAN, S.cnt2, S.lo2, Q.n, Q.irr, S.off2, W.scan_chain,
                            &ctx->d_meta->n_out, T.early_fill ? ctx->part : nullptr, log2_t2, (u32)nt_cap64 + 1));
    part_done = T.early_fill;
  } else {
    {
      Phase ph(ctx, st, GIQL_PH_COUNT, 2);
      const i64 lo_off = 1 - T.uni_len;
      hipLaunchKernelGGL(k_count_partition, dim3(cdiv((u64)S.nt2 + 1, 256)), dim3(256), 0, st,
                         sq.key[0], (u32)Q.n, Q.irr, su.key[0], (u32)U.n, U.irr, lo_off, TQ, S.nt2,
                         S.wlo2, q_mask);
      hipLaunchKernelGGL((k_range_count<RC_ITEMS_C2, RC_LDS_CAP>), dim3(S.nt2), dim3(RC_NT), 0, st,
                         sq.key[0], sq.end[0], (u32)Q.n, Q.irr, su.key[0], (u32)U.n, U.irr, lo_off,
                         S.wlo2, S.lo2, S.cnt2);
      GIQL_TRY(post_launch("range count (uniform)"));
    }
    GIQL_TRY(run_scan<u64>(ctx, st, GIQL_PH_SCAN, S.cnt2, Q.n, S.off2, W.bsums, S.off2 + Q.n, &ctx->d_meta->n_out));
  }
  if (T.early_fill) {
    const u32 nt_cap = (u32)nt_cap64;
    if (!part_done) {
      Phase ph(ctx, st, GIQL_PH_PARTITION);
      hipLaunchKernelGGL(k_partition, dim3(cdiv((u64)nt_cap + 1, 256)), dim3(256), 0, st, S.off2,
                         (u32)Q.n, (u64)0, T2, nt_cap, ctx->part, (const u64*)(S.off2 + Q.n), ctx->plan.fuse_cap);
    }
    {
      Phase ph(ctx, st, GIQL_PH_FILL);
      hipLaunchKernelGGL((k_fill<FILL_ITEMS_C2>), dim3(nt_cap), dim3(FILL_NT), 0, st, S.off2, S.lo2, sq.rid[0],
                         (u32)Q.n, su.rid[0], ctx->part, (u64)0, (u64)0, Q.out_row, U.out_row,
                         (const u64*)(S.off2 + Q.n), ctx->plan.fuse_cap);
    }
    GIQL_TRY(post_launch("fused fill"));
  }
  GIQL_TRY(read_meta(ctx, st));
  ctx->plan.n_c1 = 0;
  ctx->plan.n_reg = ctx->h_meta->n_out;
  ctx->plan.fuse_done = T.early_fill && ctx->h_meta->irr_a + ctx->h_meta->irr_b == 0 && ctx->plan.n_reg <= ctx->plan.fuse_cap;
  return GIQL_OK;
}

static int plan_general(giql_hip_ctx* ctx, hipStream_t st, int n_chrom, PlanSide& A, PlanSide& B, InnerScratch& W,
                        InnerAttempt& T) {
  InnerState& S = ctx->plan.inner;
  const LinBufs& lb = W.lb;
  SortBufs& sa = *A.sort;
  SortBufs& sbb = *B.sort;
  constexpr u32 TQ2 = RC_NT * RC_ITEMS_C2;
  const size_t n_small = A.n < B.n ? A.n : B.n;
  bind_status(W, B, A);
  const int wb_b = sort_local_bits(ctx, B.n);
  T.general_join = T.onesweep && A.out_row && T.no_irr && ctx->plan.fuse_cap > 0 && B.n >= A.n && wb_b != 0 &&
                   T.fuse_len_ok && ctx->guess.last_span > 0 &&
                   (double)A.n * ((double)(1u << (wb_b ? wb_b : 16)) + (double)ctx->h_meta->len_max_a +
                                  (double)ctx->h_meta->len_max_b) /
                           (double)ctx->guess.last_span <= 0.5 * (double)BJ_WCAP;
  SideChain sc(ctx, st, (T.onesweep && !T.general_join) ? n_small : 0);
  PlanSide* const sides[2] = {&A, &B};
  hipStream_t stream_of[2] = {A.n < B.n ? sc.stream() : st, A.n < B.n ? st : sc.stream()};
  const giql_side* keygen_of[2] = {nullptr, nullptr};
  if (T.keygen_g) keygen_of[T.big_side] = sides[T.big_side]->side;
  for (PlanSide* s : sides) {
    if (keygen_of[s->label]) {
      GIQL_TRY(span_digit_offsets(ctx, stream_of[s->label], lb, s->hist, s->gbase, nullptr, nullptr,
                                  "digit offsets (span histogram, general form)"));
    } else {
      GIQL_TRY(run_linearize(ctx, stream_of[s->label], *s->side, n_chrom, lb, s->sort->key[0], s->sort->end[0],
                             s->irr_list, s->label, 0, s->hist, s->gbase));
    }
  }
  if (T.onesweep) {
    GIQL_TRY(run_sort_onesweep(ctx, stream_of[0], sa, (u32)A.n, A.gbase, A.status, false, keygen_of[0], lb.abase, 0,
                               nullptr, T.presorted[0]));
    FuseCount fg = {};
    if (T.general_join) {
      const FuseTarget out{A.out_row, B.out_row, ctx->plan.fuse_cap};
      fg = make_fuse_count(ctx, fuse_query(A), 1, 0xFFFFFFFFu, &out, true, B.len_max,
                           reinterpret_cast<u32*>(W.scan_chain));
    }
    GIQL_TRY(run_sort_onesweep(ctx, stream_of[1], sbb, (u32)B.n, B.gbase, B.status, false, keygen_of[1], lb.abase, 0,
                               T.general_join ? &fg : nullptr, T.presorted[1]));
    GIQL_TRY(sc.join());
  } else {
    GIQL_TRY(run_sort(ctx, st, sa, (u32)A.n, W.tile_hist, W.bsums));
    GIQL_TRY(run_sort(ctx, st, sbb, (u32)B.n, W.tile_hist, W.bsums));
  }
  if (T.general_join) return finish_bucket_join(ctx, st);
  SideChain sc1(ctx, st, T.onesweep ? n_small : 0);
  hipStream_t st1 = sc1.stream();
  {
    Phase ph(ctx, st, GIQL_PH_COUNT, 4);
    if (S.c1_fill) {
      const u32 nt1r = cdiv(B.n, TQ2);
      hipLaunchKernelGGL(k_count_partition, dim3(cdiv((u64)nt1r + 1, 256)), dim3(256), 0, st1,
                         sbb.key[0], (u32)B.n, B.irr, sa.key[0], (u32)A.n, A.irr, (i64)0, TQ2, nt1r, S.wlo1);
      hipLaunchKernelGGL((k_range_count<RC_ITEMS_C2, RC_LDS_CAP>), dim3(nt1r), dim3(RC_NT), 0, st1,
                         sbb.key[0], sbb.end[0], (u32)B.n, B.irr, sa.key[0], (u32)A.n, A.irr, (i64)0, S.wlo1,
                         S.lo1, S.cnt1);
    } else {
      const u32 c1_tq = (u32)(C1_NT * S.c1_items);
      hipLaunchKernelGGL(k_count_partition, dim3(cdiv((u64)S.nt1 + 1, 256)), dim3(256), 0, st1,
                         sbb.key[0], (u32)B.n, B.irr, sa.key[0], (u32)A.n, A.irr, (i64)0, c1_tq, S.nt1,
                         S.wlo1);
      if (S.c1_items == 2)
        hipLaunchKernelGGL(k_c1_count<2>, dim3(S.nt1), dim3(C1_NT), 0, st1, sbb.key[0], sbb.end[0], (u32)B.n,
                           B.irr, sa.key[0], (u32)A.n, A.irr, S.wlo1, S.c1_base);
      else
        hipLaunchKernelGGL(k_c1_count<C1_ITEMS_MAX>, dim3(S.nt1), dim3(C1_NT), 0, st1, sbb.key[0], sbb.end[0], (u32)B.n,
                           B.irr, sa.key[0], (u32)A.n, A.irr, S.wlo1, S.c1_base);
      hipLaunchKernelGGL(k_scan_spine, dim3(1), dim3(1024), 0, st1, S.c1_base, S.nt1,
                         &ctx->d_meta->n_out_c1);
    }
    hipLaunchKernelGGL(k_count_partition, dim3(cdiv((u64)S.nt2 + 1, 256)), dim3(256), 0, st,
                       sa.key[0], (u32)A.n, A.irr, sbb.key[0], (u32)B.n, B.irr, (i64)1, TQ2, S.nt2, S.wlo2);
    hipLaunchKernelGGL((k_range_count<RC_ITEMS_C2, RC_LDS_CAP>), dim3(S.nt2), dim3(RC_NT), 0, st,
                       sa.key[0], sa.end[0], (u32)A.n, A.irr, sbb.key[0], (u32)B.n, B.irr, (i64)1, S.wlo2,
                       S.lo2, S.cnt2);
    GIQL_TRY(post_launch("range count"));
  }
  if (S.c1_fill) {
    GIQL_TRY(run_scan<u64>(ctx, st1, GIQL_PH_SCAN, S.cnt1, B.n, S.off1, W.bsums1, S.off1 + B.n, &ctx->d_meta->n_out_c1));
  }
  GIQL_TRY(run_scan<u64>(ctx, st, GIQL_PH_SCAN, S.cnt2, A.n, S.off2, W.bsums, S.off2 + A.n, &ctx->d_meta->n_out));
  GIQL_TRY(sc1.join());
  GIQL_TRY(read_meta(ctx, st));
  ctx->plan.n_c1 = ctx->h_meta->n_out_c1;
  ctx->plan.n_reg = ctx->h_meta->n_out + ctx->plan.n_c1;
  return GIQL_OK;
}

static bool settle_guesses(giql_hip_ctx* ctx, const InnerAttempt& T, size_t na, size_t nb) {
  const DevMeta& m = *ctx->h_meta;
  Guesses& g = ctx->guess;
  const bool any_irr = m.irr_a + m.irr_b > 0;
  if (T.onesweep) {
    int form;
    i64 len;
    decide_form(m, na, nb, ctx->sw.no_uniform, form, len);
    const bool aligned_now = m.aligned_ok != 0;
    const bool fuse_len_ok_now = fuse_len_ok(m, form);
    const bool form_wrong = form != T.form || len != T.uni_len;
    const bool layout_wrong = T.want_hist && !aligned_now;
    const bool coarse_wrong = T.q_skip != 0 && any_irr;
    const bool keygen_wrong = (T.keygen_g && len_min_of(m, T.big_side) <= 0) ||
                              (T.keygen_q && len_min_of(m, 1 - T.big_side) <= 0);
    const bool fuse_wrong = T.count_fused() && !fuse_len_ok_now;
    const bool sorted_wrong = (T.presorted[0] && m.unsorted_a != 0) || (T.presorted[1] && m.unsorted_b != 0);
    const bool join_wrong = T.bucket_join() && !ctx->plan.fuse_done;
    if (keygen_wrong) g.last_no_irr = false;
    g.spec_fuse_len_ok = fuse_len_ok_now;
    g.spec_sorted[0] = m.unsorted_a == 0;
    g.spec_sorted[1] = m.unsorted_b == 0;
    if (T.speculated && (form_wrong || layout_wrong || coarse_wrong || keygen_wrong || fuse_wrong || sorted_wrong ||
                         join_wrong)) {
      g.spec_valid = false;
      g.spec_misses++;
      ctx->plan.fuse_done = false;
      return false;
    }
    g.spec_valid = true;
    g.spec_form = form;
    g.spec_len = len;
    if (T.want_hist) g.spec_aligned = aligned_now;
  }
  g.last_span = m.total_span;
  g.last_no_irr = !any_irr;
  return true;
}

static int plan_irregular(giql_hip_ctx* ctx, hipStream_t st, const PlanSide& A, const PlanSide& B, InnerScratch& W) {
  const size_t nq = A.n + B.n;
  {
    Phase ph(ctx, st, GIQL_PH_IRREGULAR);
    hipLaunchKernelGGL(k_irr_count, dim3(cdiv(nq, 256)), dim3(256), 0, st, view_of(*A.side), view_of(*B.side),
                       A.irr_list, B.irr_list, ctx->d_meta, W.irr_cnt);
    GIQL_TRY(post_launch("irregular count"));
  }
  GIQL_TRY(run_scan<u64>(ctx, st, GIQL_PH_IRREGULAR, W.irr_cnt, nq, ctx->plan.irr_off, W.bsums,
                         ctx->plan.irr_off + nq));
  HIP_TRY(hipMemcpyAsync(&ctx->d_meta->n_out_irr, ctx->plan.irr_off + nq, sizeof(u64),
                         hipMemcpyDeviceToDevice, st));
  GIQL_TRY(read_meta(ctx, st));
  ctx->plan.n_irr = ctx->h_meta->n_out_irr;
  return GIQL_OK;
}

static int inner_plan_core(giql_hip_ctx* ctx, const giql_side* a, const giql_side* b,
                           int32_t n_chrom, void* stream, int64_t* n_pairs) {
  hipStream_t st = (hipStream_t)stream;
  ctx->plan.fuse_done = false;
  ctx->stats.n_a = a->n;
  ctx->stats.n_b = b->n;
  ctx->plan.side_a = *a;
  ctx->plan.side_b = *b;
  ctx->plan.n_a = (u32)a->n;
  ctx->plan.n_b = (u32)b->n;
  ctx->plan.n_chrom = n_chrom;
  ctx->plan.n_reg = ctx->plan.n_irr = ctx->plan.n_c1 = 0;
  *n_pairs = 0;
  if (a->n == 0 || b->n == 0 || n_chrom == 0) {
    ctx->plan.planned = true;
    ctx->plan.plan_is_join = false;
    return GIQL_OK;
  }
  const size_t na = (size_t)a->n, nb = (size_t)b->n;

  InnerState& S = ctx->plan.inner;
  InnerScratch W;
  InnerAttempt T;
  T.onesweep = !ctx->sw.classic_sort && na <= OS_MAX_ROWS && nb <= OS_MAX_ROWS;
  T.big_side = nb >= na ? 1 : 0;
  S.c1_items = nb <= C1_SMALL_ROWS ? 2 : C1_ITEMS_MAX;
  S.nt1 = cdiv(nb, (u32)(C1_NT * S.c1_items));
  S.c1_fill = nb <= C1_SMALL_ROWS;
  S.nt2 = cdiv(na, RC_NT * RC_ITEMS_C2);
  GIQL_TRY(claim_arena(ctx, st, [&](char* base) { return carve_inner(ctx, base, na, nb, n_chrom, T.onesweep, W); }));
  PlanSide A, B;
  A.side = a, B.side = b;
  A.n = na, B.n = nb;
  A.label = 0, B.label = 1;
  A.sort = &S.sa, B.sort = &S.sb;
  A.hist = W.hist[0], B.hist = W.hist[1];
  A.gbase = W.gbase[0], B.gbase = W.gbase[1];
  A.irr_list = ctx->plan.irr_a_list, B.irr_list = ctx->plan.irr_b_list;
  A.irr = &ctx->d_meta->irr_a, B.irr = &ctx->d_meta->irr_b;
  A.len_max = &ctx->d_meta->len_max_a, B.len_max = &ctx->d_meta->len_max_b;
  A.out_row = ctx->plan.swapped ? ctx->plan.fuse_b : ctx->plan.fuse_a;
  B.out_row = ctx->plan.swapped ? ctx->plan.fuse_a : ctx->plan.fuse_b;

  PrezeroGuard prezero_guard{ctx};
  ctx->call.first_unstable = true;
  if (T.onesweep) GIQL_TRY(zero_inner_scratch(ctx, st, W, na > nb ? na : nb));

  GIQL_TRY(begin_attempt(ctx, st, A, B, n_chrom, W, T));
  S.uniform = T.form;
  ctx->call.used_sorted[0] = T.presorted[0];
  ctx->call.used_sorted[1] = T.presorted[1];
  if (T.form == 1) {
    GIQL_TRY(plan_uniform(ctx, st, n_chrom, A, B, W, T));
  } else if (T.form == 2) {
    GIQL_TRY(plan_uniform(ctx, st, n_chrom, B, A, W, T));
  } else {
    GIQL_TRY(plan_general(ctx, st, n_chrom, A, B, W, T));
  }
  if (!settle_guesses(ctx, T, na, nb)) return GIQL_STATUS_GUESS_MISSED;
  ctx->stats.n_irregular_a = ctx->h_meta->irr_a;
  ctx->stats.n_irregular_b = ctx->h_meta->irr_b;
  ctx->stats.span = (int64_t)ctx->h_meta->total_span;

  if (ctx->h_meta->irr_a + ctx->h_meta->irr_b > 0) GIQL_TRY(plan_irregular(ctx, st, A, B, W));
  collect_spans(ctx);
  ctx->stats.reserved = S.uniform | ((T.keygen_u || T.keygen_g) ? 0x10 : 0);
  ctx->stats.n_out = (int64_t)(ctx->plan.n_reg + ctx->plan.n_irr);
  *n_pairs = (int64_t)(ctx->plan.n_reg + ctx->plan.n_irr);
  ctx->plan.planned = true;
  ctx->plan.plan_is_join = T.bucket_join();
  return GIQL_OK;
}

static int giql_hip_inner_plan_dev_impl(giql_hip_ctx* ctx, const giql_side* a, const giql_side* b,
                                        int32_t n_chrom, void* stream, int64_t* n_pairs) {
  if (!ctx || !n_pairs) return set_err(GIQL_ERR_INVALID, "ctx/n_pairs is NULL");
  GIQL_TRY(begin_pair_call(ctx, a, b, n_chrom));
  const bool swap = a->n > b->n;
  ctx->plan.swapped = swap;
  if (!swap) return inner_plan_core(ctx, a, b, n_chrom, stream, n_pairs);
  const int rc = inner_plan_core(ctx, b, a, n_chrom, stream, n_pairs);
  giql_hip_stats& stt = ctx->stats;
  const int64_t tn = stt.n_a;
  stt.n_a = stt.n_b;
  stt.n_b = tn;
  const int64_t ti = stt.n_irregular_a;
  stt.n_irregular_a = stt.n_irregular_b;
  stt.n_irregular_b = ti;
  const int form = stt.reserved & 0xF;
  if (form == 1 || form == 2) stt.reserved = (stt.reserved & ~0xF) | (3 - form);
  return rc;
}

int giql_hip_inner_plan_dev(giql_hip_ctx* ctx, const giql_side* a, const giql_side* b, int32_t n_chrom,
                            void* stream, int64_t* n_pairs) {
  return with_order_fallback(ctx, [&] { return giql_hip_inner_plan_dev_impl(ctx, a, b, n_chrom, stream, n_pairs); });
}

int giql_hip_inner_fill_dev(giql_hip_ctx* ctx, int32_t* row_a, int32_t* row_b, int64_t capacity,
                            void* stream) {
  if (!ctx) return set_err(GIQL_ERR_INVALID, "ctx is NULL");
  if (!ctx->plan.planned) return set_err(GIQL_ERR_STATE, "inner_fill without a successful inner_plan");
  const u64 total = ctx->plan.n_reg + ctx->plan.n_irr;
  if (total == 0) return GIQL_OK;
  if (ctx->plan.plan_is_join)
    return set_err(GIQL_ERR_STATE, "the last giql_hip_inner_join_dev wrote its pairs itself and kept no plan: "
                                   "call giql_hip_inner_plan_dev first");
  if (!row_a || !row_b) return set_err(GIQL_ERR_INVALID, "row_a/row_b is NULL");
  if (capacity < 0 || (u64)capacity < total)
    return set_err(GIQL_ERR_CAPACITY, "capacity %lld < %llu pairs", (long long)capacity,
                   (unsigned long long)total);
  HIP_TRY(hipSetDevice(ctx->device));
  hipStream_t st = (hipStream_t)stream;
  if (ctx->plan.swapped) {
    int32_t* t = row_a;
    row_a = row_b;
    row_b = t;
  }
  const u32 nq = ctx->plan.n_a + ctx->plan.n_b;
  InnerState& S = ctx->plan.inner;
  const u32* irr_a = &ctx->d_meta->irr_a;
  const u32* irr_b = &ctx->d_meta->irr_b;
  const u64 p1 = ctx->plan.n_c1, p2 = ctx->plan.n_reg - ctx->plan.n_c1;
  struct FillSide {
    const u32* rid;
    u32 n;
    int32_t* row;
  };
  const FillSide fa{S.sa.rid[0], ctx->plan.n_a, row_a}, fb{S.sb.rid[0], ctx->plan.n_b, row_b};
  const FillSide& Q = S.uniform != 2 ? fa : fb;
  const FillSide& U = S.uniform != 2 ? fb : fa;
  u32 nt2 = 0, nt1f = 0;
  const bool c1_fill = S.uniform == 0 && S.c1_fill && p1 > 0;
  if (p2 > 0 || c1_fill) {
    constexpr u32 T2 = FILL_NT * FILL_ITEMS_C2;
    const u64 nt2_64 = (p2 + T2 - 1) / T2, nt1_64 = c1_fill ? (p1 + T2 - 1) / T2 : 0;
    if (nt2_64 + nt1_64 > 0x7FFFFFF0ull) return set_err(GIQL_ERR_INVALID, "output too large");
    nt2 = (u32)nt2_64;
    nt1f = (u32)nt1_64;
    const size_t part_need = (size_t)nt2 + 2 + (c1_fill ? (size_t)nt1f + 2 : 0);
    GIQL_TRY(grow_part(ctx, part_need, st));
    Phase ph(ctx, st, GIQL_PH_PARTITION);
    if (p2 > 0)
      hipLaunchKernelGGL(k_partition, dim3(cdiv((u64)nt2 + 1, 256)), dim3(256), 0, st, S.off2, Q.n,
                         (u64)0, T2, nt2, ctx->part);
    if (c1_fill)
      hipLaunchKernelGGL(k_partition, dim3(cdiv((u64)nt1f + 1, 256)), dim3(256), 0, st, S.off1, ctx->plan.n_b,
                         (u64)0, T2, nt1f, ctx->part + nt2 + 2);
  }
  {
    Phase ph(ctx, st, GIQL_PH_FILL, 2);
    if (c1_fill)
      hipLaunchKernelGGL((k_fill<FILL_ITEMS_C2>), dim3(nt1f), dim3(FILL_NT), 0, st, S.off1, S.lo1, S.sb.rid[0],
                         ctx->plan.n_b, S.sa.rid[0], ctx->part + nt2 + 2, (u64)0, p1, row_b, row_a);
    else if (p1 > 0 && S.c1_items == 2)
      hipLaunchKernelGGL(k_c1_emit<2>, dim3(S.nt1), dim3(C1_NT), 0, st, S.sb.key[0], S.sb.end[0],
                         S.sb.rid[0], ctx->plan.n_b, irr_b, S.sa.key[0], S.sa.rid[0], ctx->plan.n_a, irr_a,
                         S.wlo1, S.c1_base, (u64)0, row_b, row_a);
    else if (p1 > 0)
      hipLaunchKernelGGL(k_c1_emit<C1_ITEMS_MAX>, dim3(S.nt1), dim3(C1_NT), 0, st, S.sb.key[0], S.sb.end[0],
                         S.sb.rid[0], ctx->plan.n_b, irr_b, S.sa.key[0], S.sa.rid[0], ctx->plan.n_a, irr_a,
                         S.wlo1, S.c1_base, (u64)0, row_b, row_a);
    if (p2 > 0)
      hipLaunchKernelGGL((k_fill<FILL_ITEMS_C2>), dim3(nt2), dim3(FILL_NT), 0, st, S.off2, S.lo2, Q.rid,
                         Q.n, U.rid, ctx->part, (u64)0, p2, Q.row + p1, U.row + p1);
    GIQL_TRY(post_launch("fill"));
  }
  if (ctx->plan.n_irr > 0) {
    Phase ph(ctx, st, GIQL_PH_IRREGULAR);
    hipLaunchKernelGGL(k_irr_fill, dim3(cdiv(nq, 256)), dim3(256), 0, st, view_of(ctx->plan.side_a),
                       view_of(ctx->plan.side_b), ctx->plan.irr_a_list, ctx->plan.irr_b_list, ctx->d_meta,
                       ctx->plan.irr_off, row_a + ctx->plan.n_reg, row_b + ctx->plan.n_reg);
    GIQL_TRY(post_launch("irregular fill"));
  }
  return GIQL_OK;
}

int giql_hip_inner_join_dev(giql_hip_ctx* ctx, const giql_side* a, const giql_side* b, int32_t n_chrom,
                            int32_t* row_a, int32_t* row_b, int64_t capacity, void* stream,
                            int64_t* n_pairs) {
  if (!ctx || !n_pairs) return set_err(GIQL_ERR_INVALID, "ctx/n_pairs is NULL");
  if (capacity < 0 || (capacity > 0 && (!row_a || !row_b)))
    return set_err(GIQL_ERR_INVALID, "bad output buffers");
  HIP_TRY(hipSetDevice(ctx->device));
  hipStream_t st = (hipStream_t)stream;
  {
    constexpr u32 T2 = FILL_NT * FILL_ITEMS_C2;
    const u64 nt_cap = ((u64)capacity + T2 - 1) / T2;
    if (nt_cap <= 0x7FFFFFF0ull) GIQL_TRY(grow_part(ctx, (size_t)nt_cap + 2, st));
  }
  ctx->plan.fuse_a = row_a;
  ctx->plan.fuse_b = row_b;
  ctx->plan.fuse_cap = (u64)capacity;
  const int rc = giql_hip_inner_plan_dev(ctx, a, b, n_chrom, stream, n_pairs);
  ctx->plan.fuse_a = ctx->plan.fuse_b = nullptr;
  ctx->plan.fuse_cap = 0;
  if (rc != GIQL_OK) return rc;
  if (ctx->plan.fuse_done) return GIQL_OK;
  if (*n_pairs > capacity)
    return set_err(GIQL_ERR_CAPACITY, "capacity %lld < %lld pairs", (long long)capacity, (long long)*n_pairs);
  return giql_hip_inner_fill_dev(ctx, row_a, row_b, capacity, stream);
}

struct giql_hip_index {
  int device = 0;
  u32 n = 0;
  int n_chrom = 0;
  bool general = false;
  i64 uni_len = 0;
  int len_max = 0;
  u64 span = 0;
  u32 sentinel = 0;
  int wbits = 16;
  u32 *key = nullptr, *end = nullptr, *rid = nullptr;
  u32* small = nullptr;
  size_t bytes = 0;
};

int giql_hip_index_destroy(giql_hip_index* idx) {
  if (!idx) return GIQL_OK;
  (void)hipSetDevice(idx->device);
  if (idx->key) (void)hipFree(idx->key);
  if (idx->end) (void)hipFree(idx->end);
  if (idx->rid) (void)hipFree(idx->rid);
  if (idx->small) (void)hipFree(idx->small);
  delete idx;
  return GIQL_OK;
}

int giql_hip_index_info(const giql_hip_index* idx, int64_t* n_rows, int64_t* bytes, int32_t* general, int64_t* span) {
  if (!idx) return set_err(GIQL_ERR_INVALID, "index is NULL");
  if (n_rows) *n_rows = idx->n;
  if (bytes) *bytes = (int64_t)idx->bytes;
  if (general) *general = idx->general ? 1 : 0;
  if (span) *span = (int64_t)idx->span;
  return GIQL_OK;
}

int giql_hip_index_create_dev(giql_hip_ctx* ctx, const giql_side* side, int32_t n_chrom, void* stream,
                              giql_hip_index** out) {
  if (!ctx || !out) return set_err(GIQL_ERR_INVALID, "ctx/out is NULL");
  *out = nullptr;
  GIQL_TRY(check_side(side, "side"));
  if (n_chrom < 1 || n_chrom > MM_HIST_CHROMS)
    return set_err(GIQL_ERR_STATE, "a table index takes 1..%d chromosomes (the 2^24-aligned axis), got %d", MM_HIST_CHROMS, n_chrom);
  if (side->n < 1 || (size_t)side->n > OS_MAX_ROWS) return set_err(GIQL_ERR_STATE, "a table index takes 1..2^30-1 rows");
  if (ctx->sw.classic_sort || ctx->sw.os_variant != 0 || !ctx->bucket_bnd)
    return set_err(GIQL_ERR_STATE, "this context cannot run the three-stage sort (GIQL_HIP_SORT / GIQL_HIP_OS_VARIANT)");
  GIQL_TRY(begin_call(ctx));
  hipStream_t st = (hipStream_t)stream;
  const size_t n = (size_t)side->n;
  LinBufs lb;
  SortBufs scratch;
  u32 *hist = nullptr, *gbase = nullptr, *status = nullptr;
  size_t zero_off = 0, zero_end = 0;
  auto carve = [&](char* base) {
    Carver c{base};
    common_sizes(c, n_chrom, lb);
    scratch.key[1] = c.take<u32>(n);
    scratch.end[1] = c.take<u32>(n);
    scratch.rid[1] = c.take<u32>(n);
    c.off = align_up(c.off, 256);
    zero_off = c.off;
    hist = c.take<u32>((size_t)LIN_HIST_REPLICAS * 1024);
    lb.top_partial = c.take<u32>((size_t)LIN_HIST_REPLICAS * MM_TOP_WORDS);
    gbase = c.take<u32>(1024);
    lb.abase = c.take<u32>(MM_HIST_CHROMS);
    status = c.take<u32>(3 * os_pass_words(n));
    c.off = align_up(c.off, 256);
    zero_end = c.off;
    return c.off;
// ... 2487 lines not shown
```

### giql_amd/csrc/join_kernels.hip.h

```cpp
#pragma once

#include <limits.h>

#include "dev_common.hip.h"

namespace giql {

__global__ void k_init_minmax(int* __restrict__ gmin, int* __restrict__ gmax, int n_chrom,
                              DevMeta* __restrict__ meta) {
  const int i = blockIdx.x * blockDim.x + threadIdx.x;
  if (i < n_chrom) {
    gmin[i] = INT_MAX;
    gmax[i] = INT_MIN;
  }
  if (i == 0) {
    meta->total_span = 0;
    meta->n_out = 0;
    meta->n_out_irr = 0;
    meta->n_out_c1 = 0;
    meta->sentinel = U32_MAX;
    meta->irr_a = 0;
    meta->irr_b = 0;
    meta->status = 0;
    meta->aux0 = 0;
    meta->aux1 = 0;
    meta->len_min_a = INT_MAX;
    meta->len_max_a = 0;
    meta->len_min_b = INT_MAX;
    meta->len_max_b = 0;
    meta->aligned_ok = 0;
    meta->unsorted_a = 0;
    meta->unsorted_b = 0;
    meta->inverted_a = 0;
    meta->inverted_b = 0;
  }
}

#ifndef GIQL_MM_NT
#define GIQL_MM_NT 256
#endif
#ifndef GIQL_MM_BLOCKS
#define GIQL_MM_BLOCKS 1024
#endif
#ifndef GIQL_MM_MIN_WAVES
#define GIQL_MM_MIN_WAVES 0
#endif
#if GIQL_MM_MIN_WAVES > 0
#define GIQL_MM_LAUNCH_BOUNDS(NT) __launch_bounds__(NT, GIQL_MM_MIN_WAVES)
#else
#define GIQL_MM_LAUNCH_BOUNDS(NT) __launch_bounds__(NT)
#endif
constexpr int MM_NT = GIQL_MM_NT;
constexpr int MM_NT_HIST = 2 * GIQL_MM_NT;
constexpr int MM_ITEMS = 8;
constexpr int MM_LDS_CHROMS = 4096;
constexpr int MM_MAX_BLOCKS = GIQL_MM_BLOCKS;

constexpr int LIN_HIST_REPLICAS = 64;
constexpr int MM_HIST_CHROMS = 32;
constexpr int MM_TOP_WORDS = MM_HIST_CHROMS * 256;

template <int NT>
__device__ __forceinline__ void chrom_minmax_body(const int HIST, const int* __restrict__ chrom,
                                                  const int* __restrict__ start, const int* __restrict__ end, i64 n,
                                                  int n_chrom, int* __restrict__ gmin, int* __restrict__ gmax,
                                                  DevMeta* __restrict__ meta, int len_bias, int which,
                                                  int* __restrict__ len_part, int start_off,
                                                  u32* __restrict__ hist_partial, u32* __restrict__ top_partial,
                                                  const u32 bid, const u32 nblk, u32* s_hist, u32* s_top) {
  extern __shared__ int mm_lds[];
  if (HIST) {
    for (int k = threadIdx.x; k < 3 * 256; k += NT) s_hist[k] = 0;
    for (int k = threadIdx.x; k < MM_TOP_WORDS; k += NT) s_top[k] = 0;
    __syncthreads();
  }
  const bool use_lds = n_chrom <= MM_LDS_CHROMS;
  int* lmin = use_lds ? mm_lds : gmin;
  int* lmax = use_lds ? mm_lds + n_chrom : gmax;
  if (use_lds) {
    for (int c = threadIdx.x; c < n_chrom; c += NT) {
      lmin[c] = INT_MAX;
      lmax[c] = INT_MIN;
    }
    __syncthreads();
  }
  int cur = -1, mn = INT_MAX, mx = INT_MIN;
  int lmn = INT_MAX, lmx = 0;
  bool bad = false;
  bool inv = false;
  bool neg = false;
  auto order = [&](const int c, const int s, const int pc0, const int ps0, const bool ok) {
    int pc = __builtin_amdgcn_update_dpp(0, c, 0x138, 0xF, 0xF, false);
    int ps = __builtin_amdgcn_update_dpp(0, s, 0x138, 0xF, 0xF, false);
    if (lane_id() == 0) {
      pc = pc0;
      ps = ps0;
    }
    if (ok && (pc > c || (pc == c && ps > s))) inv = true;
  };
  bool sorted_so_far = true;
  auto row = [&](const int c, const int s, const int e, const bool ok) {
    if (ok) {
      const i64 len64 = (i64)e - (i64)s + (i64)len_bias;
      const bool regular = len64 > 0;
      const int len = (int)(len64 > 0x7FFFFFF0ll ? 0x7FFFFFF0ll : len64);
      lmn = regular ? (len < lmn ? len : lmn) : 0;
      lmx = (regular && len > lmx) ? len : lmx;
      inv = inv || !regular;
      neg = neg || len64 < 0;
      if (c < 0 || c >= n_chrom) {
        bad = true;
      } else if (!sorted_so_far && use_lds) {
        const int lo = s < e ? s : e, hi = s < e ? e : s;
#if !defined(GIQL_MM_ABLATE)
        atomicMin(&mm_lds[c], lo);
        atomicMax(&mm_lds[n_chrom + c], hi);
#endif
      } else {
        if (c != cur) {
#if defined(GIQL_MM_ABLATE)
          if (cur >= 0 && (s & 0xFF) == 0) {
#else
          if (cur >= 0) {
#endif
            if (use_lds) {
              atomicMin(&mm_lds[cur], mn);
              atomicMax(&mm_lds[n_chrom + cur], mx);
            } else {
              atomicMin(&gmin[cur], mn);
              atomicMax(&gmax[cur], mx);
            }
          }
          cur = c;
          mn = INT_MAX;
          mx = INT_MIN;
        }
        const int lo = s < e ? s : e, hi = s < e ? e : s;
        mn = lo < mn ? lo : mn;
        mx = hi > mx ? hi : mx;
      }
    }
#if defined(GIQL_MM_ABLATE_HIST)
    if (HIST && (s & 0x3FF) == 0) {
#else
    if (HIST) {
#endif
      const u32 pos = (u32)(s + start_off);
      const u32 tb = ((u32)c & (MM_HIST_CHROMS - 1)) * 256u + (pos >> 24);
      if (HIST == 1 && ok) {
        atomicAdd(&s_hist[pos & 0xFFu], 1u);
        atomicAdd(&s_hist[256 + ((pos >> 8) & 0xFFu)], 1u);
      }
      if (!sorted_so_far) {
        if (ok) {
          atomicAdd(&s_hist[512 + ((pos >> 16) & 0xFFu)], 1u);
          atomicAdd(&s_top[tb], 1u);
        }
        return;
      }
      const u64 act = __ballot(ok);
      if (act != 0) {
        const u32 d2 = (pos >> 16) & 0xFFu;
        const u32 d2f = (u32)__builtin_amdgcn_readfirstlane((int)d2);
        const u32 tbf = (u32)__builtin_amdgcn_readfirstlane((int)tb);
        const bool leader = lane_id() == (u32)__ffsll((long long)act) - 1u;
        if (__ballot(ok && d2 == d2f) == act) {
          if (leader) atomicAdd(&s_hist[512 + d2f], (u32)__popcll(act));
        } else if (ok) {
          atomicAdd(&s_hist[512 + d2], 1u);
        }
        if (__ballot(ok && tb == tbf) == act) {
          if (leader) atomicAdd(&s_top[tbf], (u32)__popcll(act));
        } else if (ok) {
          atomicAdd(&s_top[tb], 1u);
        }
      }
    }
  };
  constexpr u32 TILE = 4u * NT;
  const u64 n_full = (u64)n / TILE;
  const bool vec_ok = ((((uintptr_t)chrom) | ((uintptr_t)start) | ((uintptr_t)end)) & 15u) == 0;
  typedef int mm_i4 __attribute__((ext_vector_type(4)));
  auto tile4 = [&](const u64 t, mm_i4& c4, mm_i4& s4, mm_i4& e4, int& pc, int& ps) {
    const u64 r0 = t * TILE + 4u * threadIdx.x;
    if (vec_ok) {
      c4 = ld_stream(reinterpret_cast<const mm_i4*>(chrom + r0));
      s4 = ld_stream(reinterpret_cast<const mm_i4*>(start + r0));
      e4 = ld_stream(reinterpret_cast<const mm_i4*>(end + r0));
    } else {
#pragma unroll
      for (int u = 0; u < 4; u++) {
        c4[u] = chrom[r0 + u];
        s4[u] = start[r0 + u];
        e4[u] = end[r0 + u];
      }
    }
    pc = ps = INT_MIN;
    if (lane_id() == 0 && r0 != 0) {
      pc = chrom[r0 - 1];
      ps = start[r0 - 1];
    }
  };
  auto rows4 = [&](const mm_i4& c4, const mm_i4& s4, const mm_i4& e4, const int pc0, const int ps0) {
    int pc = __builtin_amdgcn_update_dpp(0, c4[3], 0x138, 0xF, 0xF, false);
    int ps = __builtin_amdgcn_update_dpp(0, s4[3], 0x138, 0xF, 0xF, false);
    if (lane_id() == 0) {
      pc = pc0;
      ps = ps0;
    }
    if (pc > c4[0] || (pc == c4[0] && ps > s4[0])) inv = true;
#pragma unroll
    for (int u = 1; u < 4; u++)
      if (c4[u - 1] > c4[u] || (c4[u - 1] == c4[u] && s4[u - 1] > s4[u])) inv = true;
#pragma unroll
    for (int u = 0; u < 4; u++) row(c4[u], s4[u], e4[u], true);
    if (sorted_so_far) sorted_so_far = __ballot(inv) == 0ull;
  };
  {
    u64 t = bid;
    for (; t + nblk < n_full; t += 2ull * nblk) {
      mm_i4 c4a, s4a, e4a, c4b, s4b, e4b;
      int pca, psa, pcb, psb;
      tile4(t, c4a, s4a, e4a, pca, psa);
      tile4(t + nblk, c4b, s4b, e4b, pcb, psb);
      rows4(c4a, s4a, e4a, pca, psa);
      rows4(c4b, s4b, e4b, pcb, psb);
    }
    if (t < n_full) {
      mm_i4 c4a, s4a, e4a;
      int pca, psa;
      tile4(t, c4a, s4a, e4a, pca, psa);
      rows4(c4a, s4a, e4a, pca, psa);
    }
  }
  if (bid == (u32)(n_full % nblk)) {
    const u64 base = n_full * TILE;
#pragma unroll
    for (int u = 0; u < 4; u++) {
      const u64 i = base + (u64)u * NT + threadIdx.x;
      const bool ok = i < (u64)n;
      const int c_ = ok ? chrom[i] : 0, s_ = ok ? start[i] : 0;
      const bool pred = ok && i > 0 && lane_id() == 0;
      order(c_, s_, pred ? chrom[i - 1] : INT_MIN, pred ? start[i - 1] : INT_MIN, ok);
      row(c_, s_, ok ? end[i] : 0, ok);
    }
  }
  if (HIST) {
    __syncthreads();
    const size_t rep = bid % LIN_HIST_REPLICAS;
    u32* g = hist_partial + rep * 1024;
    for (int k = threadIdx.x; k < 3 * 256; k += NT) {
      const u32 v = s_hist[k];
      if (v) atomicAdd(&g[k], v);
    }
    u32* gt = top_partial + rep * MM_TOP_WORDS;
    for (int k = threadIdx.x; k < MM_TOP_WORDS; k += NT) {
      const u32 v = s_top[k];
      if (v) atomicAdd(&gt[k], v);
    }
  }
  if (cur >= 0) {
    if (use_lds) {
      atomicMin(&mm_lds[cur], mn);
      atomicMax(&mm_lds[n_chrom + cur], mx);
    } else {
      atomicMin(&gmin[cur], mn);
      atomicMax(&gmax[cur], mx);
    }
  }
  if (bad) meta->status = -4;
  if (__ballot(inv) != 0ull && lane_id() == 0) *(which ? &meta->unsorted_b : &meta->unsorted_a) = 1u;
  if (__ballot(neg) != 0ull && lane_id() == 0) *(which ? &meta->inverted_b : &meta->inverted_a) = 1u;
  {
    __shared__ int s_len[2][NT / WAVE];
    int a = lmn, b = lmx;
#pragma unroll
    for (int d = WAVE / 2; d > 0; d >>= 1) {
      const int ta = __shfl_xor(a, d, WAVE), tb = __shfl_xor(b, d, WAVE);
      a = ta < a ? ta : a;
      b = tb > b ? tb : b;
    }
    if (lane_id() == 0) {
      s_len[0][wave_id()] = a;
      s_len[1][wave_id()] = b;
    }
    __syncthreads();
    if (threadIdx.x == 0) {
#pragma unroll
      for (int k = 1; k < NT / WAVE; k++) {
        a = s_len[0][k] < a ? s_len[0][k] : a;
        b = s_len[1][k] > b ? s_len[1][k] : b;
      }
      len_part[(which * MM_MAX_BLOCKS + bid) * 2 + 0] = a;
      len_part[(which * MM_MAX_BLOCKS + bid) * 2 + 1] = b;
    }
  }
  if (use_lds) {
    __syncthreads();
    for (int c = threadIdx.x; c < n_chrom; c += NT) {
      if (lmin[c] <= lmax[c]) {
        atomicMin(&gmin[c], lmin[c]);
        atomicMax(&gmax[c], lmax[c]);
      }
    }
  }
}

template <int HIST, int NT>
__global__ GIQL_MM_LAUNCH_BOUNDS(NT) void k_chrom_minmax(const int* __restrict__ chrom,
                                                         const int* __restrict__ start,
                                                         const int* __restrict__ end, i64 n,
                                                         int n_chrom, int* __restrict__ gmin,
                                                         int* __restrict__ gmax,
                                                         DevMeta* __restrict__ meta, int len_bias,
                                                         int which, int* __restrict__ len_part,
                                                         int start_off, u32* __restrict__ hist_partial,
                                                         u32* __restrict__ top_partial) {
  __shared__ u32 s_hist[HIST ? 3 * 256 : 1];
  __shared__ u32 s_top[HIST ? MM_TOP_WORDS : 1];
  chrom_minmax_body<NT>(HIST, chrom, start, end, n, n_chrom, gmin, gmax, meta, len_bias, which, len_part, start_off,
                        hist_partial, top_partial, blockIdx.x, gridDim.x, s_hist, s_top);
}

struct MmSide {
  const int* chrom;
  const int* start;
  const int* end;
  i64 n;
  int len_bias, start_off, hist;
  u32 nblk;
  u32* hist_partial;
  u32* top_partial;
};
template <int NT>
__global__ GIQL_MM_LAUNCH_BOUNDS(NT) void k_chrom_minmax2(MmSide a, MmSide b, int n_chrom, int* __restrict__ gmin,
                                                      int* __restrict__ gmax, DevMeta* __restrict__ meta,
                                                      int* __restrict__ len_part) {
  __shared__ u32 s_hist[3 * 256];
  __shared__ u32 s_top[MM_TOP_WORDS];
  if (blockIdx.x < a.nblk)
    chrom_minmax_body<NT>(a.hist, a.chrom, a.start, a.end, a.n, n_chrom, gmin, gmax, meta, a.len_bias, 0, len_part,
                          a.start_off, a.hist_partial, a.top_partial, blockIdx.x, a.nblk, s_hist, s_top);
  else
    chrom_minmax_body<NT>(b.hist, b.chrom, b.start, b.end, b.n, n_chrom, gmin, gmax, meta, b.len_bias, 1, len_part,
                          b.start_off, b.hist_partial, b.top_partial, blockIdx.x - a.nblk, b.nblk, s_hist, s_top);
}

__global__ __launch_bounds__(256) void k_chrom_offsets(const int* __restrict__ gmin,
                                                        const int* __restrict__ gmax, int n_chrom,
                                                        int off_min, int off_max,
                                                        i64* __restrict__ chrom_base,
                                                        u32* __restrict__ chrom_first,
                                                        DevMeta* __restrict__ meta,
                                                        const int* __restrict__ len_part, int nblk_a,
                                                        int nblk_b, int want_aligned,
                                                        u32* __restrict__ abase) {
  __shared__ u64 lds[256 / WAVE + 1];
  __shared__ u64 carry_s;
  if (threadIdx.x == 0) carry_s = 0;
  if (threadIdx.x < 2 * WAVE) {
    const int which = threadIdx.x / WAVE;
    const int nblk = which ? nblk_b : nblk_a;
    int a = INT_MAX, b = 0;
    for (int k = lane_id(); k < nblk; k += WAVE) {
      const int ta = len_part[(which * MM_MAX_BLOCKS + k) * 2 + 0];
      const int tb = len_part[(which * MM_MAX_BLOCKS + k) * 2 + 1];
      a = ta < a ? ta : a;
      b = tb > b ? tb : b;
    }
#pragma unroll
    for (int d = WAVE / 2; d > 0; d >>= 1) {
      const int ta = __shfl_xor(a, d, WAVE), tb = __shfl_xor(b, d, WAVE);
      a = ta < a ? ta : a;
      b = tb > b ? tb : b;
    }
    if (lane_id() == 0) {
      if (which) {
        meta->len_min_b = a;
        meta->len_max_b = b;
      } else {
        meta->len_min_a = a;
        meta->len_max_a = b;
      }
    }
  }
  __syncthreads();
  for (int base = 0; base < n_chrom; base += 256) {
    const int c = base + threadIdx.x;
    i64 lo = 0;
    u64 span = 0;
    if (c < n_chrom && gmin[c] <= gmax[c]) {
      lo = (i64)gmin[c] + off_min;
      span = (u64)((i64)gmax[c] + off_max - lo + 1);
    }
    u64 total;
    const u64 ex = block_excl_scan<u64, 256>(span, lds, total);
    const u64 carry = carry_s;
    if (c < n_chrom) {
      chrom_base[c] = (i64)(carry + ex) - lo;
      const u64 f = carry + ex;
      chrom_first[c] = f > 0xFFFFFFFFull ? U32_MAX : (u32)f;
    }
    __syncthreads();
    if (threadIdx.x == 0) carry_s = carry + total;
    __syncthreads();
  }
  if (threadIdx.x == 0) {
    const u64 total = carry_s;
    meta->total_span = total;
    chrom_first[n_chrom] = total > 0xFFFFFFFFull ? U32_MAX : (u32)total;
    if (total > 0xFFFFFFFFull) {
      meta->status = -5;
      meta->sentinel = U32_MAX;
    } else {
      meta->sentinel = (u32)total;
    }
    if (want_aligned) {
      u32 running = 0;
      bool ok = true;
      for (int c = n_chrom; c < MM_HIST_CHROMS; c++) abase[c] = 0;
      for (int c = 0; c < n_chrom; c++) {
        abase[c] = (running & 0xFFu) << 24;
        if (gmin[c] <= gmax[c]) {
          const i64 lo = (i64)gmin[c] + off_min, hi = (i64)gmax[c] + off_max;
          if (lo < 0 || hi > 0x7FFFFFFFll) ok = false;
          const u32 nb = (u32)((hi < 0 ? 0 : hi) >> 24) + 1u;
          running += nb;
          if (running > 255u) ok = false;
        }
      }
      if (ok) {
        running = 0;
        for (int c = 0; c < n_chrom; c++) {
          chrom_base[c] = (i64)running << 24;
          chrom_first[c] = running << 24;
          if (gmin[c] <= gmax[c]) running += (u32)(((i64)gmax[c] + off_max) >> 24) + 1u;
        }
        const u64 atotal = (u64)running << 24;
        meta->total_span = atotal;
        chrom_first[n_chrom] = (u32)atotal;
        meta->sentinel = (u32)atotal;
        meta->aligned_ok = 1;
      }
    }
  }
}

__global__ __launch_bounds__(256) void k_fold_top(const u32* __restrict__ top_partial,
                                                   const u32* __restrict__ abase,
                                                   u32* __restrict__ hist_partial) {
  const u32 c = blockIdx.x, j = threadIdx.x;
  u32 sum = 0;
#pragma unroll 8
  for (int r = 0; r < LIN_HIST_REPLICAS; r++) sum += top_partial[(size_t)r * MM_TOP_WORDS + c * 256 + j];
  if (sum) atomicAdd(&hist_partial[3 * 256 + ((j + (abase[c] >> 24)) & 0xFFu)], sum);
}

__global__ __launch_bounds__(256) void k_fold_top2(const u32* __restrict__ top_a, const u32* __restrict__ top_b,
                                                    const u32* __restrict__ abase, u32* __restrict__ hist_a,
                                                    u32* __restrict__ hist_b) {
  const u32* top_partial = blockIdx.y ? top_b : top_a;
  u32* hist_partial = blockIdx.y ? hist_b : hist_a;
  const u32 c = blockIdx.x, j = threadIdx.x;
  u32 sum = 0;
#pragma unroll 8
  for (int r = 0; r < LIN_HIST_REPLICAS; r++) sum += top_partial[(size_t)r * MM_TOP_WORDS + c * 256 + j];
  if (sum) atomicAdd(&hist_partial[3 * 256 + ((j + (abase[c] >> 24)) & 0xFFu)], sum);
}

#ifndef GIQL_LIN_NT
#define GIQL_LIN_NT 256
#endif
#ifndef GIQL_LIN_BLOCKS
#define GIQL_LIN_BLOCKS 2048
#endif
constexpr int LIN_NT = GIQL_LIN_NT;
constexpr int LIN_MAX_BLOCKS = GIQL_LIN_BLOCKS;
constexpr int LIN_BASE_CAP = 1024;
#ifndef GIQL_LIN_UNROLL
#define GIQL_LIN_UNROLL 4
#endif
#ifndef GIQL_LIN_UNIFORM_FROM
#define GIQL_LIN_UNIFORM_FROM 2
#endif

template <bool END_HIST>
__global__ __launch_bounds__(LIN_NT) void k_linearize(
    const int* __restrict__ chrom, const int* __restrict__ start, const int* __restrict__ end, u32 n,
    int start_off, int end_off, int n_chrom, const i64* __restrict__ chrom_base,
    u32* __restrict__ keys, u32* __restrict__ ends, u32* __restrict__ irr_list,
    DevMeta* __restrict__ meta, int which, int keep_irregular, u32* __restrict__ hist_partial,
    u32* __restrict__ hist_partial_end) {
  __shared__ u32 s_hist[4 * 256];
  __shared__ u32 s_hist_e[END_HIST ? 4 * 256 : 1];
  __shared__ i64 s_base[LIN_BASE_CAP];
  const bool lds_base = n_chrom <= LIN_BASE_CAP;
  if (lds_base)
    for (int k = threadIdx.x; k < n_chrom; k += LIN_NT) s_base[k] = chrom_base[k];
  if (hist_partial) {
#pragma unroll
    for (int k = threadIdx.x; k < 4 * 256; k += LIN_NT) {
      s_hist[k] = 0;
      if (END_HIST) s_hist_e[k] = 0;
    }
  }
  __syncthreads();
  const u32 sentinel = meta->sentinel;
  u32* irr_count = which ? &meta->irr_b : &meta->irr_a;
  const u32 stride = gridDim.x * LIN_NT;
  const u32 n_iter = (n + stride - 1) / stride;
  constexpr int UNROLL = GIQL_LIN_UNROLL;
  const u32 i0 = blockIdx.x * LIN_NT + threadIdx.x;
  for (u32 it0 = 0; it0 < n_iter; it0 += UNROLL) {
    u32 idx[UNROLL];
    bool okv[UNROLL];
    int cv[UNROLL], sv[UNROLL], ev[UNROLL];
#pragma unroll
    for (int u = 0; u < UNROLL; u++) {
      const u64 i64_ = (u64)i0 + (u64)(it0 + u) * stride;
      okv[u] = (it0 + u) < n_iter && i64_ < n;
      idx[u] = (u32)i64_;
      cv[u] = okv[u] ? chrom[idx[u]] : 0;
      sv[u] = okv[u] ? start[idx[u]] : 0;
      ev[u] = (okv[u] && end) ? end[idx[u]] : 1;
    }
#pragma unroll
    for (int u = 0; u < UNROLL; u++) {
      if (it0 + u >= n_iter) break;
      const bool ok = okv[u];
      const u32 i = idx[u];
      bool irr = false;
      u32 k = sentinel, ke = sentinel;
      if (ok) {
        const i64 cs = (i64)sv[u] + start_off;
        const i64 ce = (i64)ev[u] + end_off;
        const int c = cv[u];
        const bool c_ok = c >= 0 && c < n_chrom;
        irr = c_ok && !keep_irregular && end != nullptr && ce <= cs;
        if (c_ok && !irr) {
          const i64 b = lds_base ? s_base[c] : chrom_base[c];
          k = (u32)(b + cs);
          ke = (u32)(b + ce);
        }
#if defined(GIQL_LIN_ABLATE) && (GIQL_LIN_ABLATE & 2)
        if (k == 0x12345u && ke == 0x54321u) keys[i] = k;
#else
        if (keys) keys[i] = k;
        if (ends) ends[i] = ke;
#endif
      }
#if defined(GIQL_LIN_ABLATE) && (GIQL_LIN_ABLATE & 1)
      if (false) {
#else
      if (hist_partial) {
#endif
        const u64 act = __ballot(ok);
#pragma unroll
        for (int p = 0; p < 4; p++) {
          const u32 d = (k >> (8 * p)) & 0xFFu;
          if (p >= GIQL_LIN_UNIFORM_FROM) {
            const u32 d0 = (u32)__builtin_amdgcn_readfirstlane((int)d);
            const u64 same = __ballot(ok && d == d0);
            if (act != 0 && same == act) {
              if (lane_id() == 0)
                atomicAdd(&s_hist[p * 256 + d0], (u32)__popcll(act));
            } else if (ok) {
              atomicAdd(&s_hist[p * 256 + d], 1u);
            }
          } else if (ok) {
            atomicAdd(&s_hist[p * 256 + d], 1u);
          }
          if (END_HIST && ok) atomicAdd(&s_hist_e[p * 256 + ((ke >> (8 * p)) & 0xFFu)], 1u);
        }
      }
      const u64 m = __ballot(irr);
      if (m) {
        u32 base = 0;
        if (lane_id() == 0) base = atomicAdd(irr_count, (u32)__popcll(m));
        base = __shfl(base, 0, WAVE);
        if (irr) irr_list[base + (u32)__popcll(m & lanemask_lt())] = i;
      }
    }
  }
  if (hist_partial) {
    __syncthreads();
    u32* g = hist_partial + (size_t)(blockIdx.x % LIN_HIST_REPLICAS) * 1024;
#pragma unroll
    for (int k = threadIdx.x; k < 4 * 256; k += LIN_NT) {
      const u32 v = s_hist[k];
      if (v) atomicAdd(&g[k], v);
      if (END_HIST) {
        const u32 ve = s_hist_e[k];
        if (ve) atomicAdd(&hist_partial_end[(size_t)(blockIdx.x % LIN_HIST_REPLICAS) * 1024 + k], ve);
      }
    }
  }
}

__global__ __launch_bounds__(LIN_NT) void k_index_query_keys(
    const int* __restrict__ chrom, const int* __restrict__ start, const int* __restrict__ end, u32 n, int start_off,
    int end_off, int n_chrom_idx, const u32* __restrict__ first, u32 sentinel, u32* __restrict__ keys,
    u32* __restrict__ ends, u32* __restrict__ dead, u32* __restrict__ irregular, int* __restrict__ len_max,
    u32* __restrict__ hist_partial) {
  __shared__ u32 s_hist[4 * 256];
  __shared__ u32 s_first[MM_HIST_CHROMS + 1];
  for (int k = threadIdx.x; k < 4 * 256; k += LIN_NT) s_hist[k] = 0;
  for (int k = threadIdx.x; k <= n_chrom_idx && k <= MM_HIST_CHROMS; k += LIN_NT) s_first[k] = first[k];
  __syncthreads();
  const u32 stride = gridDim.x * LIN_NT;
  u32 n_dead = 0;
  int lmax = 0;
  bool irr = false;
  for (u32 i = blockIdx.x * LIN_NT + threadIdx.x; i < n; i += stride) {
    const int c = chrom[i];
    const i64 cs = (i64)start[i] + start_off, ce = (i64)end[i] + end_off;
    u32 k = sentinel, ke = sentinel;
    if (c >= 0 && c < n_chrom_idx) {
      const i64 lo = (i64)s_first[c], hi = (i64)s_first[c + 1];
      if (ce <= cs) {
        irr = true;
      } else if (ce > 0 && lo + cs < hi) {
        const i64 s_ = cs < 0 ? 0 : cs;
        k = (u32)(lo + s_);
        const i64 e_ = lo + ce;
        ke = (u32)(e_ > hi ? hi : e_);
        const i64 len = (i64)ke - (i64)k;
        lmax = len > lmax ? (int)len : lmax;
      }
    }
    keys[i] = k;
    ends[i] = ke;
    if (k == sentinel) n_dead++;
#pragma unroll
    for (int p = 0; p < 4; p++) atomicAdd(&s_hist[p * 256 + ((k >> (8 * p)) & 0xFFu)], 1u);
  }
  n_dead = wave_reduce_sum(n_dead);
  lmax = (int)wave_reduce_max_u32((u32)lmax);
  if (lane_id() == 0) {
    if (n_dead) atomicAdd(dead, n_dead);
    if (lmax) atomicMax(len_max, lmax);
  }
  if (__ballot(irr) != 0ull && lane_id() == 0) *irregular = 1u;
  __syncthreads();
  u32* g = hist_partial + (size_t)(blockIdx.x % LIN_HIST_REPLICAS) * 1024;
  for (int k = threadIdx.x; k < 4 * 256; k += LIN_NT) {
    const u32 v = s_hist[k];
    if (v) atomicAdd(&g[k], v);
  }
// ... 619 lines not shown
```

### giql_amd/csrc/onesweep.hip.h

```cpp
#pragma once

#include "dev_common.hip.h"

namespace giql {

constexpr int OS_BINS = 256;
constexpr int OS_MIN_TILE = 4096;
constexpr u32 OS_FLAG_AGG = 1u << 30;
constexpr u32 OS_FLAG_PREFIX = 2u << 30;
constexpr u32 OS_VALUE_MASK = (1u << 30) - 1u;
constexpr u32 OS_MAX_ROWS = (1u << 30) - 1u;
constexpr u32 OS_NO_TILE = 0xFFFFFFFFu;
#ifndef GIQL_OS_LB_WIDTH
#define GIQL_OS_LB_WIDTH 8
#endif
constexpr int OS_LB_WIDTH = GIQL_OS_LB_WIDTH;
#ifndef GIQL_OS_PRESTAGE
#define GIQL_OS_PRESTAGE 1
#endif

constexpr u32 OS_HELP_AFTER = 1u << 11;

#if defined(GIQL_OS_TIMELINE)
constexpr u32 OS_TL_TILES = 1u << 15;
__device__ unsigned long long g_os_tl[OS_TL_TILES * 16];
#define GIQL_TL(tile, k)                                                             \
  do {                                                                               \
    if (threadIdx.x == 0 && (tile) < OS_TL_TILES) g_os_tl[(size_t)(tile) * 16 + (k)] = wall_clock64(); \
  } while (0)
#else
#define GIQL_TL(tile, k) do { } while (0)
#endif

__device__ __forceinline__ void wave_match8(u32 d, u64 active, u32& below, u32& total) {
  u32 mis_lo = 0, mis_hi = 0;
#pragma unroll
  for (int b = 0; b < 8; b++) {
    const int s = __builtin_amdgcn_sbfe((int)d, b, 1);
    const u64 m = __ballot(s != 0);
    mis_lo |= (u32)m ^ (u32)s;
    mis_hi |= (u32)(m >> 32) ^ (u32)s;
  }
  const u32 p_lo = (u32)active & ~mis_lo;
  const u32 p_hi = (u32)(active >> 32) & ~mis_hi;
  below = __builtin_amdgcn_mbcnt_hi(p_hi, __builtin_amdgcn_mbcnt_lo(p_lo, 0u));
  total = (u32)__popc(p_lo) + (u32)__popc(p_hi);
}

#ifndef GIQL_OS_XCD_GROUP
#define GIQL_OS_XCD_GROUP 16
#endif
constexpr u32 OS_GROUPS = XCD_GROUPS;
constexpr u32 OS_GROUP = GIQL_OS_XCD_GROUP;

__device__ __forceinline__ u32 os_tile_of_ticket(u32 t, u32 n_tiles) { return xcd_tile_of_block<OS_GROUP>(t, n_tiles); }

__device__ __forceinline__ void os_store(u32* p, u32 v) { *p = v; }

template <int PAYLOAD, int OS_NT, int OS_ITEMS, bool FULL, bool KEYGEN = false>
__device__ __forceinline__ u32 onesweep_tile(
    const u32* __restrict__ keys_in, const u32* __restrict__ ends_in, const u32* __restrict__ rids_in,
    u32* __restrict__ keys_out, u32* __restrict__ ends_out, u32* __restrict__ rids_out, u32 n_valid,
    u32 tile, u32 tile_base, int shift, const u32* __restrict__ gbase, u32* __restrict__ status,
    DevMeta* __restrict__ meta, u32* s_buf, u32 (*s_wcnt)[OS_BINS], u32* s_dstart, u32* s_goff,
    u32* s_scan, u32* s_help, u32 help_after, u32 n_total, const u32* s_abase = nullptr, u32 start_off = 0,
    u32 end_off = 0, const bool unstable = false) {
  constexpr int OS_NW = OS_NT / WAVE;
  const u32 tid = threadIdx.x;
  const u32 lane = lane_id();
  const u32 w = wave_id();

  u32 key[OS_ITEMS];
  const u32 wbase = w * (OS_ITEMS * WAVE);
  const u32* kin = keys_in + tile_base;
  const u32* ein = (PAYLOAD & 2) ? ends_in + tile_base : nullptr;
  const u32* rin = ((PAYLOAD & 1) && rids_in && !KEYGEN) ? rids_in + tile_base : nullptr;
  const int* cin = KEYGEN ? reinterpret_cast<const int*>((PAYLOAD & 2) ? rids_in : ends_in) + tile_base : nullptr;
  if (KEYGEN) {
    u32 cc[OS_ITEMS];
#pragma unroll
    for (int i = 0; i < OS_ITEMS; i++) {
      const u32 r = wbase + i * WAVE + lane;
      const bool ok = FULL || r < n_valid;
      cc[i] = ok ? (u32)cin[r] : 0u;
      key[i] = ok ? kin[r] : 0u;
    }
    __syncthreads();
#pragma unroll
    for (int i = 0; i < OS_ITEMS; i++) {
      const u32 r = wbase + i * WAVE + lane;
      const bool ok = FULL || r < n_valid;
      key[i] = ok ? s_abase[cc[i] & 31u] + key[i] + start_off : U32_MAX;
    }
  } else {
#pragma unroll
    for (int i = 0; i < OS_ITEMS; i++) {
      const u32 r = wbase + i * WAVE + lane;
      const bool ok = FULL || r < n_valid;
      key[i] = ok ? kin[r] : U32_MAX;
    }
    __syncthreads();
  }

  GIQL_TL(tile, 1);
#if defined(GIQL_OS_TIMELINE)
  __builtin_amdgcn_s_waitcnt(0);
  GIQL_TL(tile, 2);
#endif
  u32 rank[OS_ITEMS];
  if (unstable) {
    u32* wcnt = s_wcnt[w];
#pragma unroll
    for (int i = 0; i < OS_ITEMS; i++) {
      const u32 r = wbase + i * WAVE + lane;
      const bool ok = FULL || r < n_valid;
      rank[i] = ok ? atomicAdd(&wcnt[(key[i] >> shift) & 0xFFu], 1u) : 0u;
    }
  } else {
    u32* wcnt = s_wcnt[w];
#pragma unroll
    for (int i = 0; i < OS_ITEMS; i++) {
      const u32 r = wbase + i * WAVE + lane;
      const bool ok = FULL || r < n_valid;
      const u32 d = (key[i] >> shift) & 0xFFu;
      const u64 active = FULL ? ~0ull : __ballot(ok);
      u32 below, total;
#if defined(GIQL_ABLATE) && GIQL_ABLATE == 2
      below = lane;
      total = 64;
      (void)active;
#else
      wave_match8(d, active, below, total);
#endif
      rank[i] = 0;
      if (ok) {
        const u32 pre = wcnt[d];
        rank[i] = pre + below;
        if (below == 0) wcnt[d] = pre + total;
      }
    }
  }
  GIQL_TL(tile, 3);
  __syncthreads();
  GIQL_TL(tile, 4);

  u32 lb_count = 0;
#if defined(GIQL_OS_FAKE_SEG)
  u32 lb_fake = 0;
#endif
  if (tid < OS_BINS) {
    u32 run = 0;
#pragma unroll
    for (int k = 0; k < OS_NW; k++) {
      const u32 c = s_wcnt[k][tid];
      s_wcnt[k][tid] = run;
      run += c;
    }
    const u32 count = run;
    lb_count = count;
    GIQL_TL(tile, 5);
    const u32 incl = wave_incl_scan(count);
    if (lane == WAVE - 1) s_scan[w] = incl;
#if !(defined(GIQL_ABLATE) && GIQL_ABLATE == 1)
#if defined(GIQL_OS_FAKE_SEG)
    {
      const u32 n_tiles_ = (n_total + (u32)(OS_NT * OS_ITEMS) - 1u) / (u32)(OS_NT * OS_ITEMS);
      const u32 bin_ = (tid == OS_BINS - 1 ? n_total : gbase[tid + 1]) - gbase[tid];
      const u32 fake_ = (u32)((u64)bin_ * tile / n_tiles_);
      const bool head_ = (tile % GIQL_OS_FAKE_SEG) == 0;
      lb_fake = head_ ? fake_ : 0u;
      __hip_atomic_store(status + (size_t)tile * OS_BINS + tid,
                         (head_ ? OS_FLAG_PREFIX : OS_FLAG_AGG) | ((count + lb_fake) & OS_VALUE_MASK), __ATOMIC_RELAXED,
                         __HIP_MEMORY_SCOPE_AGENT);
    }
#else
    __hip_atomic_store(status + (size_t)tile * OS_BINS + tid, (tile == 0 ? OS_FLAG_PREFIX : OS_FLAG_AGG) | count,
                       __ATOMIC_RELAXED, __HIP_MEMORY_SCOPE_AGENT);
#endif
#endif
    s_dstart[tid] = incl - count;
  }
  __syncthreads();
  if (tid < OS_BINS) {
    u32 wb = 0;
#pragma unroll
    for (int k = 0; k < OS_BINS / WAVE; k++)
      if (k < (int)w) wb += s_scan[k];
    s_dstart[tid] += wb;
  }
  __syncthreads();
  GIQL_TL(tile, 6);

  u32 pos[OS_ITEMS];
#pragma unroll
  for (int i = 0; i < OS_ITEMS; i++) {
    const u32 d = (key[i] >> shift) & 0xFFu;
    pos[i] = s_dstart[d] + s_wcnt[w][d] + rank[i];
  }
  u32 pay[OS_ITEMS];
  if (PAYLOAD & 2) {
#pragma unroll
    for (int i = 0; i < OS_ITEMS; i++) {
      const u32 r = wbase + i * WAVE + lane;
      if (KEYGEN)
        pay[i] = (FULL || r < n_valid) ? s_abase[(u32)cin[r] & 31u] + ein[r] + end_off : 0u;
      else
        pay[i] = (FULL || r < n_valid) ? ein[r] : 0u;
    }
  } else if (PAYLOAD & 1) {
#pragma unroll
    for (int i = 0; i < OS_ITEMS; i++) {
      const u32 r = wbase + i * WAVE + lane;
      pay[i] = (FULL || r < n_valid) ? (rin ? rin[r] : tile_base + r) : 0u;
    }
  }
#pragma unroll
  for (int i = 0; i < OS_ITEMS; i++) {
    const u32 r = wbase + i * WAVE + lane;
    if (FULL || r < n_valid) s_buf[pos[i]] = key[i];
  }
  GIQL_TL(tile, 7);
  constexpr bool PRESTAGE = GIQL_OS_PRESTAGE && (PAYLOAD == 1 || PAYLOAD == 2);
  u32 ks[PRESTAGE ? OS_ITEMS : 1], ps[PRESTAGE ? OS_ITEMS : 1];
  if (PRESTAGE) {
    __syncthreads();
#pragma unroll
    for (int i = 0; i < OS_ITEMS; i++) {
      const u32 p = i * OS_NT + tid;
      ks[i] = (FULL || p < n_valid) ? s_buf[p] : 0u;
    }
    __syncthreads();
#pragma unroll
    for (int i = 0; i < OS_ITEMS; i++) {
      const u32 r = wbase + i * WAVE + lane;
      if (FULL || r < n_valid) s_buf[pos[i]] = pay[i];
    }
    __syncthreads();
#pragma unroll
    for (int i = 0; i < OS_ITEMS; i++) {
      const u32 p = i * OS_NT + tid;
      ps[i] = (FULL || p < n_valid) ? s_buf[p] : 0u;
    }
  }
  GIQL_TL(tile, 8);
  if (tid < OS_BINS) {
    u32 excl = 0;
#if defined(GIQL_OS_FAKE_SEG)
    excl = lb_fake;
#endif
#if defined(GIQL_ABLATE) && GIQL_ABLATE == 1
    excl = tile * 32;
#else
#if defined(GIQL_OS_FAKE_SEG)
    if ((tile % GIQL_OS_FAKE_SEG) != 0) {
#else
    if (tile != 0) {
#endif
      u32* st = status + (size_t)tile * OS_BINS + tid;
      const u32 count = lb_count;
      u32 t = tile;
      u32 spins = 0;
      bool done = false;
#if defined(GIQL_OS_TIMELINE)
      u32 tl_polls = 0;
#endif
      while (!done) {
#if defined(GIQL_OS_TIMELINE)
        tl_polls++;
#endif
        u32 v[OS_LB_WIDTH];
#pragma unroll
        for (int j = 0; j < OS_LB_WIDTH; j++) {
          const u32 tj = t > (u32)j ? t - 1 - j : 0u;
          v[j] = __hip_atomic_load(status + (size_t)tj * OS_BINS + tid, __ATOMIC_RELAXED,
                                   __HIP_MEMORY_SCOPE_AGENT);
        }
        int used = 0;
#pragma unroll
        for (int j = 0; j < OS_LB_WIDTH; j++) {
          if (done || used != j) continue;
          if (t <= (u32)j) {
            done = true;
            continue;
          }
          const u32 f = v[j] >> 30;
          if (f == 0) continue;
          excl += v[j] & OS_VALUE_MASK;
          used = j + 1;
          if (f == 2u) done = true;
        }
        t -= (u32)used;
        if (!done && used == 0) {
          if (++spins > help_after) {
            atomicMin(s_help, t - 1u);
            break;
          }
          __builtin_amdgcn_s_sleep(1);
        }
        if (t == 0) done = true;
      }
      if (done)
        __hip_atomic_store(st, OS_FLAG_PREFIX | ((excl + count) & OS_VALUE_MASK), __ATOMIC_RELAXED,
                           __HIP_MEMORY_SCOPE_AGENT);
#if defined(GIQL_OS_TIMELINE)
      if (tid == 0 && tile < OS_TL_TILES) {
        g_os_tl[(size_t)tile * 16 + 12] = tl_polls;
        g_os_tl[(size_t)tile * 16 + 13] = tile - t;
      }
#endif
    }
#endif
    s_goff[tid] = gbase[tid] + excl - s_dstart[tid];
  }
  GIQL_TL(tile, 9);
  __syncthreads();
  {
    const u32 help = *s_help;
    if (help != OS_NO_TILE) return help;
  }
#if defined(GIQL_ABLATE) && GIQL_ABLATE == 3
  if (key[0] != 0x12345u) return OS_NO_TILE;
#endif
  if (PRESTAGE) {
    u32* pout = (PAYLOAD & 2) ? ends_out : rids_out;
#pragma unroll
    for (int i = 0; i < OS_ITEMS; i++) {
      const u32 p = i * OS_NT + tid;
      if (FULL || p < n_valid) {
        const u32 d = s_goff[(ks[i] >> shift) & 0xFFu] + p;
        os_store(keys_out + d, ks[i]);
        os_store(pout + d, ps[i]);
      }
    }
    GIQL_TL(tile, 10);
#if defined(GIQL_OS_TIMELINE)
    __builtin_amdgcn_s_waitcnt(0);
    GIQL_TL(tile, 11);
#endif
    return OS_NO_TILE;
  }
  u32 dst[OS_ITEMS];
#pragma unroll
  for (int i = 0; i < OS_ITEMS; i++) {
    const u32 p = i * OS_NT + tid;
    dst[i] = 0;
    if (FULL || p < n_valid) {
      const u32 k = s_buf[p];
      dst[i] = s_goff[(k >> shift) & 0xFFu] + p;
      os_store(keys_out + dst[i], k);
    }
  }
  GIQL_TL(tile, 9);
  if (PAYLOAD == 3) {
    u32 pay2[OS_ITEMS];
#pragma unroll
    for (int i = 0; i < OS_ITEMS; i++) {
      const u32 r = wbase + i * WAVE + lane;
      pay2[i] = (FULL || r < n_valid) ? (rin ? rin[r] : tile_base + r) : 0u;
    }
    __syncthreads();
#pragma unroll
    for (int i = 0; i < OS_ITEMS; i++) {
      const u32 r = wbase + i * WAVE + lane;
      if (FULL || r < n_valid) s_buf[pos[i]] = pay[i];
    }
    __syncthreads();
#pragma unroll
    for (int i = 0; i < OS_ITEMS; i++) {
      const u32 p = i * OS_NT + tid;
      if (FULL || p < n_valid) os_store(ends_out + dst[i], s_buf[p]);
    }
    __syncthreads();
#pragma unroll
    for (int i = 0; i < OS_ITEMS; i++) {
      const u32 r = wbase + i * WAVE + lane;
      if (FULL || r < n_valid) s_buf[pos[i]] = pay2[i];
    }
    __syncthreads();
#pragma unroll
    for (int i = 0; i < OS_ITEMS; i++) {
      const u32 p = i * OS_NT + tid;
      if (FULL || p < n_valid) os_store(rids_out + dst[i], s_buf[p]);
    }
  } else if (PAYLOAD != 0) {
    u32* out = (PAYLOAD & 2) ? ends_out : rids_out;
    __syncthreads();
#pragma unroll
    for (int i = 0; i < OS_ITEMS; i++) {
      const u32 r = wbase + i * WAVE + lane;
      if (FULL || r < n_valid) s_buf[pos[i]] = pay[i];
    }
    __syncthreads();
#pragma unroll
    for (int i = 0; i < OS_ITEMS; i++) {
      const u32 p = i * OS_NT + tid;
      if (FULL || p < n_valid) os_store(out + dst[i], s_buf[p]);
    }
  }
  GIQL_TL(tile, 10);
#if defined(GIQL_OS_TIMELINE)
  __builtin_amdgcn_s_waitcnt(0);
  GIQL_TL(tile, 11);
#endif
  return OS_NO_TILE;
}

template <int PAYLOAD, int OS_NT, int OS_ITEMS, bool KEYGEN = false>
__device__ __forceinline__ u32 os_run_tile(
    const u32* __restrict__ keys_in, const u32* __restrict__ ends_in, const u32* __restrict__ rids_in,
    u32* __restrict__ keys_out, u32* __restrict__ ends_out, u32* __restrict__ rids_out, u32 n, u32 tile,
    int shift, const u32* __restrict__ gbase, u32* __restrict__ status, DevMeta* __restrict__ meta,
    u32* s_buf, u32 (*s_wcnt)[OS_BINS], u32* s_dstart, u32* s_goff, u32* s_scan, u32* s_help,
    u32 help_after, const u32* s_abase = nullptr, u32 start_off = 0, u32 end_off = 0, const bool unstable = false) {
  constexpr int OS_TILE = OS_NT * OS_ITEMS;
  const u32 tile_base = tile * OS_TILE;
  const u32 n_valid = (n - tile_base) < (u32)OS_TILE ? (n - tile_base) : (u32)OS_TILE;
  if (n_valid == (u32)OS_TILE)
    return onesweep_tile<PAYLOAD, OS_NT, OS_ITEMS, true, KEYGEN>(keys_in, ends_in, rids_in, keys_out, ends_out,
                                                                 rids_out, n_valid, tile, tile_base, shift, gbase,
                                                                 status, meta, s_buf, s_wcnt, s_dstart, s_goff,
                                                                 s_scan, s_help, help_after, n, s_abase, start_off, end_off,
                                                                 unstable);
  return onesweep_tile<PAYLOAD, OS_NT, OS_ITEMS, false, KEYGEN>(keys_in, ends_in, rids_in, keys_out, ends_out,
                                                                rids_out, n_valid, tile, tile_base, shift, gbase,
                                                                status, meta, s_buf, s_wcnt, s_dstart, s_goff,
                                                                s_scan, s_help, help_after, n, s_abase, start_off, end_off,
                                                                unstable);
}

template <int PAYLOAD, int OS_NT, int OS_ITEMS, bool KEYGEN = false>
__device__ __noinline__ void os_help_loop(
    const u32* __restrict__ keys_in, const u32* __restrict__ ends_in, const u32* __restrict__ rids_in,
    u32* __restrict__ keys_out, u32* __restrict__ ends_out, u32* __restrict__ rids_out, u32 n, u32 own,
    u32 need, int shift, const u32* __restrict__ gbase, u32* __restrict__ status,
    DevMeta* __restrict__ meta, u32* s_buf, u32 (*s_wcnt)[OS_BINS], u32* s_dstart, u32* s_goff,
    u32* s_scan, u32* s_help, u32 help_after, const u32* s_abase = nullptr, u32 start_off = 0, u32 end_off = 0,
    const bool unstable = false) {
  constexpr int OS_NW = OS_NT / WAVE;
  const u32 tid = threadIdx.x;
  u32 cur = need;
  for (u32 rounds = 0;; rounds++) {
    __syncthreads();
#pragma unroll
    for (int k = tid; k < OS_NW * OS_BINS; k += OS_NT) (&s_wcnt[0][0])[k] = 0;
    if (tid == 0) *s_help = OS_NO_TILE;
    __syncthreads();
    const u32 r = os_run_tile<PAYLOAD, OS_NT, OS_ITEMS, KEYGEN>(keys_in, ends_in, rids_in, keys_out, ends_out,
                                                               rids_out, n, cur, shift, gbase, status, meta, s_buf,
                                                               s_wcnt, s_dstart, s_goff, s_scan, s_help, help_after,
                                                               s_abase, start_off, end_off, unstable);
    if (r == OS_NO_TILE) {
      if (cur == own) return;
      cur = own;
    } else {
      cur = r;
      if (rounds > (1u << 20)) {
        if (tid == 0) meta->status = -2;
        return;
      }
    }
  }
}

template <int PAYLOAD, int OS_NT, int OS_ITEMS, bool KEYGEN = false>
__global__ __launch_bounds__(OS_NT, (OS_NT == 1024 && (PAYLOAD != 3 || OS_ITEMS <= 8)) ? 8 : 1) void k_onesweep(
    const u32* __restrict__ keys_in, const u32* __restrict__ ends_in, const u32* __restrict__ rids_in,
    u32* __restrict__ keys_out, u32* __restrict__ ends_out, u32* __restrict__ rids_out, u32 n,
    int shift, const u32* __restrict__ gbase, u32* __restrict__ status, u32* __restrict__ ticket,
    DevMeta* __restrict__ meta, int order, u32 help_after, const u32* __restrict__ abase = nullptr,
    u32 start_off = 0, u32 end_off = 0, int unstable = 0) {
  constexpr int OS_TILE = OS_NT * OS_ITEMS;
  constexpr int OS_NW = OS_NT / WAVE;
  __shared__ u32 s_buf[OS_TILE];
  __shared__ u32 s_wcnt[OS_NW][OS_BINS];
  __shared__ u32 s_dstart[OS_BINS];
  __shared__ u32 s_goff[OS_BINS];
  __shared__ u32 s_scan[OS_BINS / WAVE + 1];
  __shared__ u32 s_tile;
  __shared__ u32 s_help;
  __shared__ u32 s_abase[KEYGEN ? 32 : 1];

  const u32 tid = threadIdx.x;
  if (KEYGEN && tid < 32) s_abase[tid] = abase[tid];
  if (tid == 0) {
    if (order != 2) s_tile = atomicAdd(ticket, 1u);
    s_help = OS_NO_TILE;
  }
#pragma unroll
  for (int k = tid; k < OS_NW * OS_BINS; k += OS_NT) (&s_wcnt[0][0])[k] = 0;
  if (order != 2) __syncthreads();
  const u32 own = order == 2 ? xcd_tile_of_block<OS_GROUP>(blockIdx.x, gridDim.x) : s_tile;
  if (own * OS_TILE >= n) return;
  GIQL_TL(own, 0);
  const u32 need = os_run_tile<PAYLOAD, OS_NT, OS_ITEMS, KEYGEN>(keys_in, ends_in, rids_in, keys_out, ends_out,
                                                                rids_out, n, own, shift, gbase, status, meta, s_buf,
                                                                s_wcnt, s_dstart, s_goff, s_scan, &s_help, help_after,
                                                                s_abase, start_off, end_off, unstable != 0);
  if (need != OS_NO_TILE)
    os_help_loop<PAYLOAD, OS_NT, OS_ITEMS, KEYGEN>(keys_in, ends_in, rids_in, keys_out, ends_out, rids_out, n, own,
                                                   need, shift, gbase, status, meta, s_buf, s_wcnt, s_dstart,
                                                   s_goff, s_scan, &s_help, help_after, s_abase, start_off, end_off,
                                                   unstable != 0);
}

template <int PAYLOAD>
__global__ __launch_bounds__(256) void k_keygen_stream(const int* __restrict__ chrom, const int* __restrict__ start,
                                                        const int* __restrict__ end, u32 n,
                                                        const u32* __restrict__ abase, u32 start_off, u32 end_off,
                                                        u32* __restrict__ keys, u32* __restrict__ ends,
                                                        u32* __restrict__ rids) {
  __shared__ u32 s_abase[32];
  if (threadIdx.x < 32) s_abase[threadIdx.x] = abase[threadIdx.x];
  __syncthreads();
  const u32 stride = gridDim.x * 256u;
  for (u32 i = blockIdx.x * 256u + threadIdx.x; i < n; i += stride) {
    const u32 b = s_abase[(u32)chrom[i] & 31u];
    keys[i] = b + (u32)start[i] + start_off;
    if (PAYLOAD & 2) ends[i] = b + (u32)end[i] + end_off;
    if (PAYLOAD & 1) rids[i] = i;
  }
}

__global__ __launch_bounds__(256) void k_iota(u32* __restrict__ out, u32 n) {
  const u32 stride = gridDim.x * 256u;
  for (u32 i = blockIdx.x * 256u + threadIdx.x; i < n; i += stride) out[i] = i;
}

}
```

Before: 193.5 billion.

## Move big-side interval length check from span pass into keygen sort pass

When the plan is speculated to have a uniform interval length on the big side, the span/minmax kernel stops reading the end column for that side and substitutes a fixed length. The length min/max validation moves into the first onesweep keygen pass, which reads end alongside start and chrom and reduces per-tile min/max into device metadata via atomics. This removes one full pass over the big side's end array. The cost is extra loads and reductions in the sort pass, and a new speculation-miss condition when the observed lengths differ from the guess.

New measurement: 189.7 billion. -2.0%, worse.

```diff
diff --git a/giql_amd/csrc/giql_hip.hip b/giql_amd/csrc/giql_hip.hip
--- a/giql_amd/csrc/giql_hip.hip
+++ b/giql_amd/csrc/giql_hip.hip
@@ -105,6 +105,7 @@
   int inject_timeout = 0;
   bool no_uniform = false;
   bool no_span_hist = false;
+  bool no_sort_len = false;
   bool no_coarse_b = false;
   double coarse_max_group_rows = 8.0;
   bool no_fuse_count = false;
@@ -458,7 +459,8 @@
 static inline bool sort_is_local(const giql_hip_ctx* ctx, size_t n) { return sort_local_bits(ctx, n) != 0; }
 
 static int run_spans(giql_hip_ctx* ctx, hipStream_t st, const giql_side& a, const giql_side& b,
-                     int n_chrom, const LinBufs& lb, int hist_side = -1, u32* hist_partial = nullptr) {
+                     int n_chrom, const LinBufs& lb, int hist_side = -1, u32* hist_partial = nullptr,
+                     int noend_side = -1, int noend_len = 0) {
   const bool hist = hist_side >= 0 && hist_partial && lb.abase && lb.top_partial &&
                     n_chrom <= MM_HIST_CHROMS && (hist_side ? b.n : a.n) > 0;
   const bool hist2 = hist && lb.hist_partial2 && lb.top_partial2 && ctx->call.prezeroed && (hist_side ? a.n : b.n) > 0;
@@ -467,6 +469,9 @@
     HIP_TRY(hipMemsetAsync(lb.top_partial, 0, (size_t)LIN_HIST_REPLICAS * MM_TOP_WORDS * sizeof(u32), st));
   }
   Phase ph(ctx, st, GIQL_PH_SPAN, 4);
+  if (!(a.n > 0 && b.n > 0)) noend_side = -1;
+  ctx->stats.phase_bytes[GIQL_PH_SPAN] +=
+      (int64_t)12 * ((int64_t)a.n + (int64_t)b.n) - (noend_side < 0 ? 0 : (int64_t)4 * (noend_side ? b.n : a.n));
   hipLaunchKernelGGL(k_init_minmax, dim3(cdiv((u64)n_chrom + 1, 256)), dim3(256), 0, st, lb.gmin,
                      lb.gmax, n_chrom, ctx->d_meta);
   const size_t lds = n_chrom <= MM_LDS_CHROMS ? (size_t)n_chrom * 2 * sizeof(int) : 0;
@@ -492,12 +497,18 @@
       ms[k].len_bias = s.end_off - s.start_off;
       ms[k].start_off = with_hist ? s.start_off : 0;
       ms[k].hist = !with_hist ? 0 : (sort_local_bits(ctx, (size_t)s.n) == 16 ? 2 : 1);
+      ms[k].fixed_len = k == noend_side ? noend_len : 0;
       ms[k].nblk = grid;
       ms[k].hist_partial = with_hist ? hp : nullptr;
       ms[k].top_partial = with_hist ? (k == hist_side ? lb.top_partial : lb.top_partial2) : nullptr;
     }
-    hipLaunchKernelGGL((k_chrom_minmax2<MM_NT_HIST>), dim3(ms[0].nblk + ms[1].nblk), dim3(MM_NT_HIST), lds, st, ms[0], ms[1],
-                       n_chrom, lb.gmin, lb.gmax, ctx->d_meta, lb.len_part);
+#define GIQL_MM2_LAUNCH(NA, NB)                                                                                  \
+  hipLaunchKernelGGL((k_chrom_minmax2<MM_NT_HIST, NA, NB>), dim3(ms[0].nblk + ms[1].nblk), dim3(MM_NT_HIST), lds, st, \
+                     ms[0], ms[1], n_chrom, lb.gmin, lb.gmax, ctx->d_meta, lb.len_part)
+    if (noend_side == 0) GIQL_MM2_LAUNCH(true, false);
+    else if (noend_side == 1) GIQL_MM2_LAUNCH(false, true);
+    else GIQL_MM2_LAUNCH(false, false);
+#undef GIQL_MM2_LAUNCH
   } else
   for (int k = 0; k < 2; k++) {
     const giql_side& s = *sides[k];
@@ -692,7 +703,8 @@
 static int run_sort_onesweep(giql_hip_ctx* ctx, hipStream_t st, SortBufs& sb, u32 n,
                              const u32* gbase, u32* status, bool keep_rids = false,
                              const giql_side* keygen = nullptr, const u32* abase = nullptr,
-                             int skip_digits = 0, const FuseCount* fuse = nullptr, bool presorted = false) {
+                             int skip_digits = 0, const FuseCount* fuse = nullptr, bool presorted = false,
+                             int* len_out = nullptr) {
   if (n == 0) return GIQL_OK;
   if (presorted) {
     const int mode = (sb.rid[0] ? 1 : 0) | (sb.end[0] ? 2 : 0);
@@ -740,7 +752,7 @@
       const u32* gb = gbase + digit * OS_BINS;
       {
         const int w_out = 1 + (sb.rid[0] ? 1 : 0) + (sb.end[0] ? 1 : 0);
-        const int w_in = (pass == 0 && keygen) ? 2 + (sb.end[0] ? 1 : 0)
+        const int w_in = (pass == 0 && keygen) ? 2 + ((sb.end[0] || len_out) ? 1 : 0)
                                                : 1 + ((sb.rid[0] && !first) ? 1 : 0) + (sb.end[0] ? 1 : 0);
         ctx->stats.phase_bytes[GIQL_PH_SORT_SCATTER] += (int64_t)4 * (w_in + w_out) * n;
       }
@@ -754,6 +766,12 @@
                              reinterpret_cast<const u32*>(keygen->chrom), sb.key[dst], sb.end[dst], sb.rid[dst], n,
                              digit * 8, gb, stat, claim, ctx->d_meta, ctx->guess.os_order, ctx->sw.os_help_after, abase,
                              (u32)keygen->start_off, (u32)keygen->end_off, unstable);
+        else if (len_out)
+          hipLaunchKernelGGL((k_onesweep<1, 1024, 8, true, true>), dim3(grid), dim3(1024), 0, st,
+                             reinterpret_cast<const u32*>(keygen->start), reinterpret_cast<const u32*>(keygen->chrom),
+                             reinterpret_cast<const u32*>(keygen->end), sb.key[dst], (u32*)nullptr, sb.rid[dst], n,
+                             digit * 8, gb, stat, claim, ctx->d_meta, ctx->guess.os_order, ctx->sw.os_help_after, abase,
+                             (u32)keygen->start_off, 0u, unstable, len_out, keygen->end_off - keygen->start_off);
         else
           hipLaunchKernelGGL((k_onesweep<1, 1024, 8, true>), dim3(grid), dim3(1024), 0, st,
                              reinterpret_cast<const u32*>(keygen->start), reinterpret_cast<const u32*>(keygen->chrom),
@@ -1028,6 +1046,7 @@
       {"GIQL_HIP_INJECT_TIMEOUT", parse_int, &s.inject_timeout},
       {"GIQL_HIP_NO_UNIFORM", parse_flag, &s.no_uniform},
       {"GIQL_HIP_NO_SPAN_HIST", parse_flag, &s.no_span_hist},
+      {"GIQL_HIP_NO_SORT_LEN", parse_flag, &s.no_sort_len},
       {"GIQL_HIP_NO_COARSE_B", parse_flag, &s.no_coarse_b},
       {"GIQL_HIP_COARSE_MAX_GROUP_ROWS", parse_positive, &s.coarse_max_group_rows},
       {"GIQL_HIP_NO_FUSE_COUNT", parse_flag, &s.no_fuse_count},
@@ -1187,6 +1206,7 @@
   bool keygen_u = false;
   bool keygen_q = false;
   bool keygen_g = false;
+  bool len_in_sort = false;
   bool presorted[2] = {false, false};
   bool no_irr = false;
   bool fuse_len_ok = false;
@@ -1312,7 +1332,12 @@
     W.lb.hist_partial2 = other.hist;
     W.lb.top_partial2 = W.top_partial_q;
   }
-  GIQL_TRY(run_spans(ctx, st, *A.side, *B.side, n_chrom, W.lb, T.want_hist ? T.big_side : -1, big.hist));
+  const i64 raw_len = g.spec_len - (i64)(big.side->end_off - big.side->start_off);
+  T.len_in_sort = T.speculated && T.want_hist && g.spec_form == big_form && g.spec_len > 0 && raw_len > 0 &&
+                  raw_len <= 0x7FFFFFF0ll && !g.spec_sorted[T.big_side] && !ctx->sw.no_sort_len && other.n > 0 &&
+                  big.n > 0;
+  GIQL_TRY(run_spans(ctx, st, *A.side, *B.side, n_chrom, W.lb, T.want_hist ? T.big_side : -1, big.hist,
+                     T.len_in_sort ? T.big_side : -1, (int)raw_len));
   if (T.speculated) {
     T.form = g.spec_form;
     T.uni_len = g.spec_len;
@@ -1450,8 +1475,9 @@
     fc.dev.lo_out = S.lo2;
     fc.dev.hi_out = S.cnt2;
   }
+  int* const len_out = T.len_in_sort ? (U.label ? &ctx->d_meta->len_min_b : &ctx->d_meta->len_min_a) : nullptr;
   GIQL_TRY(run_sort_onesweep(ctx, st, su, (u32)U.n, U.gbase, U.status, false, T.keygen_u ? U.side : nullptr, lb.abase,
-                             0, T.fuse_cnt ? &fc : nullptr, T.presorted[U.label]));
+                             0, T.fuse_cnt ? &fc : nullptr, T.presorted[U.label], len_out));
   GIQL_TRY(sc.join());
   constexpr u32 TQ = RC_NT * RC_ITEMS_C2;
   S.nt2 = cdiv(Q.n, TQ);
@@ -1606,12 +1632,13 @@
     const bool fuse_wrong = T.count_fused() && !fuse_len_ok_now;
     const bool sorted_wrong = (T.presorted[0] && m.unsorted_a != 0) || (T.presorted[1] && m.unsorted_b != 0);
     const bool join_wrong = T.bucket_join() && !ctx->plan.fuse_done;
+    const bool len_wrong = T.len_in_sort && (len_min_of(m, T.big_side) != T.uni_len || len_max_of(m, T.big_side) != T.uni_len);
     if (keygen_wrong) g.last_no_irr = false;
     g.spec_fuse_len_ok = fuse_len_ok_now;
     g.spec_sorted[0] = m.unsorted_a == 0;
     g.spec_sorted[1] = m.unsorted_b == 0;
     if (T.speculated && (form_wrong || layout_wrong || coarse_wrong || keygen_wrong || fuse_wrong || sorted_wrong ||
-                         join_wrong)) {
+                         join_wrong || len_wrong)) {
       g.spec_valid = false;
       g.spec_misses++;
       ctx->plan.fuse_done = false;
diff --git a/giql_amd/csrc/join_kernels.hip.h b/giql_amd/csrc/join_kernels.hip.h
--- a/giql_amd/csrc/join_kernels.hip.h
+++ b/giql_amd/csrc/join_kernels.hip.h
@@ -60,14 +60,15 @@
 constexpr int MM_HIST_CHROMS = 32;
 constexpr int MM_TOP_WORDS = MM_HIST_CHROMS * 256;
 
-template <int NT>
+template <int NT, bool NOEND = false>
 __device__ __forceinline__ void chrom_minmax_body(const int HIST, const int* __restrict__ chrom,
                                                   const int* __restrict__ start, const int* __restrict__ end, i64 n,
                                                   int n_chrom, int* __restrict__ gmin, int* __restrict__ gmax,
                                                   DevMeta* __restrict__ meta, int len_bias, int which,
                                                   int* __restrict__ len_part, int start_off,
                                                   u32* __restrict__ hist_partial, u32* __restrict__ top_partial,
-                                                  const u32 bid, const u32 nblk, u32* s_hist, u32* s_top) {
+                                                  const u32 bid, const u32 nblk, u32* s_hist, u32* s_top,
+                                                  const int fixed_len = 0) {
   extern __shared__ int mm_lds[];
   if (HIST) {
     for (int k = threadIdx.x; k < 3 * 256; k += NT) s_hist[k] = 0;
@@ -99,15 +100,18 @@
     if (ok && (pc > c || (pc == c && ps > s))) inv = true;
   };
   bool sorted_so_far = true;
-  auto row = [&](const int c, const int s, const int e, const bool ok) {
+  auto row = [&](const int c, const int s, const int e_in, const bool ok) {
+    const int e = NOEND ? (int)((u32)s + (u32)fixed_len) : e_in;
     if (ok) {
-      const i64 len64 = (i64)e - (i64)s + (i64)len_bias;
-      const bool regular = len64 > 0;
-      const int len = (int)(len64 > 0x7FFFFFF0ll ? 0x7FFFFFF0ll : len64);
-      lmn = regular ? (len < lmn ? len : lmn) : 0;
-      lmx = (regular && len > lmx) ? len : lmx;
-      inv = inv || !regular;
-      neg = neg || len64 < 0;
+      if (!NOEND) {
+        const i64 len64 = (i64)e - (i64)s + (i64)len_bias;
+        const bool regular = len64 > 0;
+        const int len = (int)(len64 > 0x7FFFFFF0ll ? 0x7FFFFFF0ll : len64);
+        lmn = regular ? (len < lmn ? len : lmn) : 0;
+        lmx = (regular && len > lmx) ? len : lmx;
+        inv = inv || !regular;
+        neg = neg || len64 < 0;
+      }
       if (c < 0 || c >= n_chrom) {
         bad = true;
       } else if (!sorted_so_far && use_lds) {
@@ -179,22 +183,23 @@
   };
   constexpr u32 TILE = 4u * NT;
   const u64 n_full = (u64)n / TILE;
-  const bool vec_ok = ((((uintptr_t)chrom) | ((uintptr_t)start) | ((uintptr_t)end)) & 15u) == 0;
+  const bool vec_ok = ((((uintptr_t)chrom) | ((uintptr_t)start) | (NOEND ? (uintptr_t)0 : (uintptr_t)end)) & 15u) == 0;
   typedef int mm_i4 __attribute__((ext_vector_type(4)));
   auto tile4 = [&](const u64 t, mm_i4& c4, mm_i4& s4, mm_i4& e4, int& pc, int& ps) {
     const u64 r0 = t * TILE + 4u * threadIdx.x;
     if (vec_ok) {
       c4 = ld_stream(reinterpret_cast<const mm_i4*>(chrom + r0));
       s4 = ld_stream(reinterpret_cast<const mm_i4*>(start + r0));
-      e4 = ld_stream(reinterpret_cast<const mm_i4*>(end + r0));
+      if (!NOEND) e4 = ld_stream(reinterpret_cast<const mm_i4*>(end + r0));
     } else {
 #pragma unroll
       for (int u = 0; u < 4; u++) {
         c4[u] = chrom[r0 + u];
         s4[u] = start[r0 + u];
-        e4[u] = end[r0 + u];
-      }
-    }
+        if (!NOEND) e4[u] = end[r0 + u];
+      }
+    }
+    if (NOEND) e4 = mm_i4{0, 0, 0, 0};
     pc = ps = INT_MIN;
     if (lane_id() == 0 && r0 != 0) {
       pc = chrom[r0 - 1];
@@ -242,7 +247,7 @@
       const int c_ = ok ? chrom[i] : 0, s_ = ok ? start[i] : 0;
       const bool pred = ok && i > 0 && lane_id() == 0;
       order(c_, s_, pred ? chrom[i - 1] : INT_MIN, pred ? start[i - 1] : INT_MIN, ok);
-      row(c_, s_, ok ? end[i] : 0, ok);
+      row(c_, s_, (ok && !NOEND) ? end[i] : 0, ok);
     }
   }
   if (HIST) {
@@ -328,22 +333,25 @@
   const int* end;
   i64 n;
   int len_bias, start_off, hist;
+  int fixed_len;
   u32 nblk;
   u32* hist_partial;
   u32* top_partial;
 };
-template <int NT>
+template <int NT, bool NOEND_A = false, bool NOEND_B = false>
 __global__ GIQL_MM_LAUNCH_BOUNDS(NT) void k_chrom_minmax2(MmSide a, MmSide b, int n_chrom, int* __restrict__ gmin,
                                                       int* __restrict__ gmax, DevMeta* __restrict__ meta,
                                                       int* __restrict__ len_part) {
   __shared__ u32 s_hist[3 * 256];
   __shared__ u32 s_top[MM_TOP_WORDS];
   if (blockIdx.x < a.nblk)
-    chrom_minmax_body<NT>(a.hist, a.chrom, a.start, a.end, a.n, n_chrom, gmin, gmax, meta, a.len_bias, 0, len_part,
-                          a.start_off, a.hist_partial, a.top_partial, blockIdx.x, a.nblk, s_hist, s_top);
+    chrom_minmax_body<NT, NOEND_A>(a.hist, a.chrom, a.start, a.end, a.n, n_chrom, gmin, gmax, meta, a.len_bias, 0,
+                                   len_part, a.start_off, a.hist_partial, a.top_partial, blockIdx.x, a.nblk, s_hist,
+                                   s_top, a.fixed_len);
   else
-    chrom_minmax_body<NT>(b.hist, b.chrom, b.start, b.end, b.n, n_chrom, gmin, gmax, meta, b.len_bias, 1, len_part,
-                          b.start_off, b.hist_partial, b.top_partial, blockIdx.x - a.nblk, b.nblk, s_hist, s_top);
+    chrom_minmax_body<NT, NOEND_B>(b.hist, b.chrom, b.start, b.end, b.n, n_chrom, gmin, gmax, meta, b.len_bias, 1,
+                                   len_part, b.start_off, b.hist_partial, b.top_partial, blockIdx.x - a.nblk, b.nblk,
+                                   s_hist, s_top, b.fixed_len);
 }
 
 __global__ __launch_bounds__(256) void k_chrom_offsets(const int* __restrict__ gmin,
diff --git a/giql_amd/csrc/onesweep.hip.h b/giql_amd/csrc/onesweep.hip.h
--- a/giql_amd/csrc/onesweep.hip.h
+++ b/giql_amd/csrc/onesweep.hip.h
@@ -57,14 +57,16 @@
 
 __device__ __forceinline__ void os_store(u32* p, u32 v) { *p = v; }
 
-template <int PAYLOAD, int OS_NT, int OS_ITEMS, bool FULL, bool KEYGEN = false>
+template <int PAYLOAD, int OS_NT, int OS_ITEMS, bool FULL, bool KEYGEN = false, bool LENCHK = false>
 __device__ __forceinline__ u32 onesweep_tile(
     const u32* __restrict__ keys_in, const u32* __restrict__ ends_in, const u32* __restrict__ rids_in,
     u32* __restrict__ keys_out, u32* __restrict__ ends_out, u32* __restrict__ rids_out, u32 n_valid,
     u32 tile, u32 tile_base, int shift, const u32* __restrict__ gbase, u32* __restrict__ status,
     DevMeta* __restrict__ meta, u32* s_buf, u32 (*s_wcnt)[OS_BINS], u32* s_dstart, u32* s_goff,
     u32* s_scan, u32* s_help, u32 help_after, u32 n_total, const u32* s_abase = nullptr, u32 start_off = 0,
-    u32 end_off = 0, const bool unstable = false) {
+    u32 end_off = 0, const bool unstable = false, int* __restrict__ len_out = nullptr, int len_bias = 0,
+    u32* s_len = nullptr) {
+  static_assert(!LENCHK || (KEYGEN && PAYLOAD == 1 && OS_NT > OS_BINS), "LENCHK: a (key, rid) KEYGEN pass");
   constexpr int OS_NW = OS_NT / WAVE;
   const u32 tid = threadIdx.x;
   const u32 lane = lane_id();
@@ -78,19 +80,40 @@
   const int* cin = KEYGEN ? reinterpret_cast<const int*>((PAYLOAD & 2) ? rids_in : ends_in) + tile_base : nullptr;
   if (KEYGEN) {
     u32 cc[OS_ITEMS];
+    u32 ee[LENCHK ? OS_ITEMS : 1];
+    const int* lin = LENCHK ? reinterpret_cast<const int*>(rids_in) + tile_base : nullptr;
 #pragma unroll
     for (int i = 0; i < OS_ITEMS; i++) {
       const u32 r = wbase + i * WAVE + lane;
       const bool ok = FULL || r < n_valid;
       cc[i] = ok ? (u32)cin[r] : 0u;
       key[i] = ok ? kin[r] : 0u;
-    }
-    __syncthreads();
+      if (LENCHK) ee[i] = ok ? (u32)lin[r] : 0u;
+    }
+    __syncthreads();
+    u32 dmin = U32_MAX, dmax = 0u;
 #pragma unroll
     for (int i = 0; i < OS_ITEMS; i++) {
       const u32 r = wbase + i * WAVE + lane;
       const bool ok = FULL || r < n_valid;
+      if (LENCHK && ok) {
+        const u32 d = (int)ee[i] > (int)key[i] ? ee[i] - key[i] : 0u;
+        dmin = d < dmin ? d : dmin;
+        dmax = d > dmax ? d : dmax;
+      }
       key[i] = ok ? s_abase[cc[i] & 31u] + key[i] + start_off : U32_MAX;
+    }
+    if (LENCHK) {
+#pragma unroll
+      for (int d = WAVE / 2; d > 0; d >>= 1) {
+        const u32 ta = __shfl_xor(dmin, d, WAVE), tb = __shfl_xor(dmax, d, WAVE);
+        dmin = ta < dmin ? ta : dmin;
+        dmax = tb > dmax ? tb : dmax;
+      }
+      if (lane == 0) {
+        s_len[w] = dmin;
+        s_len[OS_NW + w] = dmax;
+      }
     }
   } else {
 #pragma unroll
@@ -148,6 +171,21 @@
 #if defined(GIQL_OS_FAKE_SEG)
   u32 lb_fake = 0;
 #endif
+  if (LENCHK && tid == OS_BINS) {
+    u32 mn = U32_MAX, mx = 0u;
+#pragma unroll
+    for (int k = 0; k < OS_NW; k++) {
+      mn = s_len[k] < mn ? s_len[k] : mn;
+      mx = s_len[OS_NW + k] > mx ? s_len[OS_NW + k] : mx;
+    }
+    auto canon = [&](const u32 d) {
+      const i64 v = d ? (i64)d + (i64)len_bias : 0;
+      return (int)(v < 0 ? 0 : (v > 0x7FFFFFF0ll ? 0x7FFFFFF0ll : v));
+    };
+    const int cmn = canon(mn), cmx = canon(mx);
+    if (cmn < __hip_atomic_load(&len_out[0], __ATOMIC_RELAXED, __HIP_MEMORY_SCOPE_AGENT)) atomicMin(&len_out[0], cmn);
+    if (cmx > __hip_atomic_load(&len_out[1], __ATOMIC_RELAXED, __HIP_MEMORY_SCOPE_AGENT)) atomicMax(&len_out[1], cmx);
+  }
   if (tid < OS_BINS) {
     u32 run = 0;
 #pragma unroll
@@ -405,37 +443,36 @@
   return OS_NO_TILE;
 }
 
-template <int PAYLOAD, int OS_NT, int OS_ITEMS, bool KEYGEN = false>
+template <int PAYLOAD, int OS_NT, int OS_ITEMS, bool KEYGEN = false, bool LENCHK = false>
 __device__ __forceinline__ u32 os_run_tile(
     const u32* __restrict__ keys_in, const u32* __restrict__ ends_in, const u32* __restrict__ rids_in,
     u32* __restrict__ keys_out, u32* __restrict__ ends_out, u32* __restrict__ rids_out, u32 n, u32 tile,
     int shift, const u32* __restrict__ gbase, u32* __restrict__ status, DevMeta* __restrict__ meta,
     u32* s_buf, u32 (*s_wcnt)[OS_BINS], u32* s_dstart, u32* s_goff, u32* s_scan, u32* s_help,
-    u32 help_after, const u32* s_abase = nullptr, u32 start_off = 0, u32 end_off = 0, const bool unstable = false) {
+    u32 help_after, const u32* s_abase = nullptr, u32 start_off = 0, u32 end_off = 0, const bool unstable = false,
+    int* __restrict__ len_out = nullptr, int len_bias = 0, u32* s_len = nullptr) {
   constexpr int OS_TILE = OS_NT * OS_ITEMS;
   const u32 tile_base = tile * OS_TILE;
   const u32 n_valid = (n - tile_base) < (u32)OS_TILE ? (n - tile_base) : (u32)OS_TILE;
   if (n_valid == (u32)OS_TILE)
-    return onesweep_tile<PAYLOAD, OS_NT, OS_ITEMS, true, KEYGEN>(keys_in, ends_in, rids_in, keys_out, ends_out,
-                                                                 rids_out, n_valid, tile, tile_base, shift, gbase,
-                                                                 status, meta, s_buf, s_wcnt, s_dstart, s_goff,
-                                                                 s_scan, s_help, help_after, n, s_abase, start_off, end_off,
-                                                                 unstable);
-  return onesweep_tile<PAYLOAD, OS_NT, OS_ITEMS, false, KEYGEN>(keys_in, ends_in, rids_in, keys_out, ends_out,
-                                                                rids_out, n_valid, tile, tile_base, shift, gbase,
-                                                                status, meta, s_buf, s_wcnt, s_dstart, s_goff,
-                                                                s_scan, s_help, help_after, n, s_abase, start_off, end_off,
-                                                                unstable);
-}
-
-template <int PAYLOAD, int OS_NT, int OS_ITEMS, bool KEYGEN = false>
+    return onesweep_tile<PAYLOAD, OS_NT, OS_ITEMS, true, KEYGEN, LENCHK>(
+        keys_in, ends_in, rids_in, keys_out, ends_out, rids_out, n_valid, tile, tile_base, shift, gbase, status, meta,
+        s_buf, s_wcnt, s_dstart, s_goff, s_scan, s_help, help_after, n, s_abase, start_off, end_off, unstable, len_out,
+        len_bias, s_len);
+  return onesweep_tile<PAYLOAD, OS_NT, OS_ITEMS, false, KEYGEN, LENCHK>(
+      keys_in, ends_in, rids_in, keys_out, ends_out, rids_out, n_valid, tile, tile_base, shift, gbase, status, meta,
+      s_buf, s_wcnt, s_dstart, s_goff, s_scan, s_help, help_after, n, s_abase, start_off, end_off, unstable, len_out,
+      len_bias, s_len);
+}
+
+template <int PAYLOAD, int OS_NT, int OS_ITEMS, bool KEYGEN = false, bool LENCHK = false>
 __device__ __noinline__ void os_help_loop(
     const u32* __restrict__ keys_in, const u32* __restrict__ ends_in, const u32* __restrict__ rids_in,
     u32* __restrict__ keys_out, u32* __restrict__ ends_out, u32* __restrict__ rids_out, u32 n, u32 own,
     u32 need, int shift, const u32* __restrict__ gbase, u32* __restrict__ status,
     DevMeta* __restrict__ meta, u32* s_buf, u32 (*s_wcnt)[OS_BINS], u32* s_dstart, u32* s_goff,
     u32* s_scan, u32* s_help, u32 help_after, const u32* s_abase = nullptr, u32 start_off = 0, u32 end_off = 0,
-    const bool unstable = false) {
+    const bool unstable = false, int* __restrict__ len_out = nullptr, int len_bias = 0, u32* s_len = nullptr) {
   constexpr int OS_NW = OS_NT / WAVE;
   const u32 tid = threadIdx.x;
   u32 cur = need;
@@ -445,10 +482,9 @@
     for (int k = tid; k < OS_NW * OS_BINS; k += OS_NT) (&s_wcnt[0][0])[k] = 0;
     if (tid == 0) *s_help = OS_NO_TILE;
     __syncthreads();
-    const u32 r = os_run_tile<PAYLOAD, OS_NT, OS_ITEMS, KEYGEN>(keys_in, ends_in, rids_in, keys_out, ends_out,
-                                                               rids_out, n, cur, shift, gbase, status, meta, s_buf,
-                                                               s_wcnt, s_dstart, s_goff, s_scan, s_help, help_after,
-                                                               s_abase, start_off, end_off, unstable);
+    const u32 r = os_run_tile<PAYLOAD, OS_NT, OS_ITEMS, KEYGEN, LENCHK>(
+        keys_in, ends_in, rids_in, keys_out, ends_out, rids_out, n, cur, shift, gbase, status, meta, s_buf, s_wcnt,
+        s_dstart, s_goff, s_scan, s_help, help_after, s_abase, start_off, end_off, unstable, len_out, len_bias, s_len);
     if (r == OS_NO_TILE) {
       if (cur == own) return;
       cur = own;
@@ -462,13 +498,13 @@
   }
 }
 
-template <int PAYLOAD, int OS_NT, int OS_ITEMS, bool KEYGEN = false>
+template <int PAYLOAD, int OS_NT, int OS_ITEMS, bool KEYGEN = false, bool LENCHK = false>
 __global__ __launch_bounds__(OS_NT, (OS_NT == 1024 && (PAYLOAD != 3 || OS_ITEMS <= 8)) ? 8 : 1) void k_onesweep(
     const u32* __restrict__ keys_in, const u32* __restrict__ ends_in, const u32* __restrict__ rids_in,
     u32* __restrict__ keys_out, u32* __restrict__ ends_out, u32* __restrict__ rids_out, u32 n,
     int shift, const u32* __restrict__ gbase, u32* __restrict__ status, u32* __restrict__ ticket,
     DevMeta* __restrict__ meta, int order, u32 help_after, const u32* __restrict__ abase = nullptr,
-    u32 start_off = 0, u32 end_off = 0, int unstable = 0) {
+    u32 start_off = 0, u32 end_off = 0, int unstable = 0, int* __restrict__ len_out = nullptr, int len_bias = 0) {
   constexpr int OS_TILE = OS_NT * OS_ITEMS;
   constexpr int OS_NW = OS_NT / WAVE;
   __shared__ u32 s_buf[OS_TILE];
@@ -479,6 +515,7 @@
   __shared__ u32 s_tile;
   __shared__ u32 s_help;
   __shared__ u32 s_abase[KEYGEN ? 32 : 1];
+  __shared__ u32 s_len[LENCHK ? 2 * OS_NW : 1];
 
   const u32 tid = threadIdx.x;
   if (KEYGEN && tid < 32) s_abase[tid] = abase[tid];
@@ -492,15 +529,15 @@
   const u32 own = order == 2 ? xcd_tile_of_block<OS_GROUP>(blockIdx.x, gridDim.x) : s_tile;
   if (own * OS_TILE >= n) return;
   GIQL_TL(own, 0);
-  const u32 need = os_run_tile<PAYLOAD, OS_NT, OS_ITEMS, KEYGEN>(keys_in, ends_in, rids_in, keys_out, ends_out,
-                                                                rids_out, n, own, shift, gbase, status, meta, s_buf,
-                                                                s_wcnt, s_dstart, s_goff, s_scan, &s_help, help_after,
-                                                                s_abase, start_off, end_off, unstable != 0);
+  const u32 need = os_run_tile<PAYLOAD, OS_NT, OS_ITEMS, KEYGEN, LENCHK>(
+      keys_in, ends_in, rids_in, keys_out, ends_out, rids_out, n, own, shift, gbase, status, meta, s_buf, s_wcnt,
+      s_dstart, s_goff, s_scan, &s_help, help_after, s_abase, start_off, end_off, unstable != 0, len_out, len_bias,
+      s_len);
   if (need != OS_NO_TILE)
-    os_help_loop<PAYLOAD, OS_NT, OS_ITEMS, KEYGEN>(keys_in, ends_in, rids_in, keys_out, ends_out, rids_out, n, own,
-                                                   need, shift, gbase, status, meta, s_buf, s_wcnt, s_dstart,
-                                                   s_goff, s_scan, &s_help, help_after, s_abase, start_off, end_off,
-                                                   unstable != 0);
+    os_help_loop<PAYLOAD, OS_NT, OS_ITEMS, KEYGEN, LENCHK>(
+        keys_in, ends_in, rids_in, keys_out, ends_out, rids_out, n, own, need, shift, gbase, status, meta, s_buf,
+        s_wcnt, s_dstart, s_goff, s_scan, &s_help, help_after, s_abase, start_off, end_off, unstable != 0, len_out,
+        len_bias, s_len);
 }
 
 template <int PAYLOAD>
```
